# ubiquity6/MVSNet

Hardware: AMD Instinct MI355X
Metric: depth maps/sec (N=5, D=192, 160x128) (higher is better)
Workload: dtype f32; 1 GPU; M: features->depth, N=5 views, D=192 planes, 160x128 feature maps, C=32, 3D-CNN regulariser (RegNetUS0), network_mode=normal; one reference view per step per GPU, sharded by reference view; conv_impl=auto, streams_per_gpu=1

## Files before the change

include/mvsnet_hip.h:

```cpp
#ifndef MVSNET_HIP_H_
#define MVSNET_HIP_H_

#include <stddef.h>
#include <stdint.h>

#ifdef __cplusplus
extern "C" {
#endif

#define MVS_ABI_VERSION 1

#define MVS_E_BADARG   (-1)
#define MVS_E_SHAPE    (-2)
#define MVS_E_WORKSPACE (-3)
#define MVS_E_NOT_PREPARED (-4)
#define MVS_E_NO_SLOT  (-5)

#define MVS_CONV_IMPL_AUTO   0
#define MVS_CONV_IMPL_SCALAR 1
#define MVS_CONV_IMPL_MFMA   2
#define MVS_CONV_IMPL_BF16X3 3

int mvs_abi_version(void);
const char* mvs_error_string(int code);
int mvs_set_conv_impl(int impl);
int mvs_get_conv_impl(void);

#define MVS_HOOK_CV_TILE_ROWS_LOG2    0
#define MVS_HOOK_CONV_NO_SPAN         1
#define MVS_HOOK_CONV_NO_FUSE2        2
#define MVS_HOOK_S2_PLANES            3
#define MVS_HOOK_GRU_ONE_STREAM       4
#define MVS_HOOK_GRU_PRODUCER_THREADS 5
#define MVS_HOOK_UNET_PERSISTENT       6
#define MVS_HOOK_UNET_GRID            7
#define MVS_HOOK_FUSE2_PLANES          8
#define MVS_HOOK_REGNET_SIDE_BRANCH    9
#define MVS_HOOK_OUT_PLANES           10
#define MVS_HOOK_BN_SLOTS             11
#define MVS_HOOK_PAIR_SLOTS           12
#define MVS_HOOK_CONV_FULL_SWEEPS     13
#define MVS_HOOK_PAIR_PLANES          14
#define MVS_HOOK_S1_PLANES            15
#define MVS_HOOK_SPAN_FORCE           16
#define MVS_HOOK_PAIR_DIRECT          17
#define MVS_HOOK_PAIR_WAVES4          18
#define MVS_HOOK_COUNT                19
int mvs_set_test_hook(int id, int value);
int mvs_get_test_hook(int id);

int mvs_homography_transforms_f32(const float* cams, int view_num, int depth_num,
                                  float depth_start, float depth_interval, float depth_end,
                                  int inverse_depth, float* homographies, float* transforms,
                                  void* stream);

int mvs_cost_volume_f32(const float* ref, const float* src, const float* transforms,
                        int view_num, int depth_total, int d_begin, int d_count,
                        int H, int W, int C, int variant, int negate, int border,
                        float* cost, void* stream);

int mvs_warp_f32(const float* image, const float* transform8, int H, int W, int C, int border,
                 float* out, void* stream);

int mvs_conv3d_f32(const float* x, const float* x_scale, const float* x_shift,
                   const float* x2, const float* x2_scale, const float* x2_shift,
                   const float* w, int D, int H, int W, int Cin, int Cout, int stride,
                   float* y, double* stats, void* stream);
int mvs_deconv3d_f32(const float* x, const float* x_scale, const float* x_shift,
                     const float* x2, const float* x2_scale, const float* x2_shift,
                     const float* w, int D, int H, int W, int Cin, int Cout,
                     float* y, double* stats, void* stream);

int mvs_conv3d_pair_f32(const float* x, const float* w1, const float* w2, int D, int H, int W,
                        int Cin, int Cout1, int Cout2, float* y1, double* stats1,
                        float* y2, double* stats2, void* stream);

int mvs_bn_finalize_f32(const double* stats, int C, double count, const float* gamma,
                        const float* beta, float eps, float* scale, float* shift, void* stream);
int mvs_zero_f64(double* p, size_t n, void* stream);

size_t mvs_regnet_workspace_bytes(int D, int H, int W, int cin, int base);
size_t mvs_regnet_prepared_floats(int cin, int base);
int mvs_regnet_prepare_f32(const float* const* weights, int cin, int base, float* prepared,
                           void* stream);
int mvs_regnet_us0_prepared_f32(const float* cost, int D, int H, int W, int cin, int base,
                                const float* const* weights, const float* prepared,
                                const float* const* gammas, const float* const* betas, float eps,
                                void* workspace, size_t workspace_bytes, float* reg, void* stream);

int mvs_gn_stat_slots(void);
size_t mvs_conv2d_prepared_floats(int ks, int cin1, int cin2, int cout);
int mvs_conv2d_prepare_f32(const float* w, int ks, int cin1, int cin2, int cout, float* prepared, void* stream);
int mvs_conv2d_prepare_dgrad_f32(const float* w, int ks, int cin_fwd, int cout_fwd, float* prepared, void* stream);
int mvs_conv2d_gn_f32(const float* x1, const double* stats1, const float* gamma1, const float* beta1, int c1, int relu1,
                      const float* x2, const double* stats2, const float* gamma2, const float* beta2, int c2, int relu2,
                      const float* prepared, int V, int H, int W, int cout, int ks, int stride,
                      float* y, double* stats_out, void* stream);
int mvs_unet_prepare_many_f32(int n, const int* kind, const float* const* w, const int* ks, const int* c1, const int* c2,
                              const int* cin_src, const int* cout, float* const* prepared, void* stream);
size_t mvs_deconv2d_prepared_floats(int cin, int cout);
int mvs_deconv2d_prepare_f32(const float* w, int cin, int cout, float* prepared, void* stream);
int mvs_deconv2d_gn_f32(const float* x, const double* stats, const float* gamma, const float* beta, int cin, int relu,
                        const float* w, const float* prepared, int V, int H, int W, int cout, float* y,
                        double* stats_out, void* stream);

size_t mvs_center_images_workspace_bytes(int V);
int mvs_center_images_u8_f32(const uint8_t* images, int V, int H, int W, float* out4, void* workspace, void* stream);

int mvs_profile_dominant(int enable);
int mvs_profile_dominant_ms(double* avg_ms, int* count);
int mvs_profile_stages(int enable);
int mvs_profile_stages_ms(double* avg_ms3, int* count);
int mvs_profile_layers(int enable);
int mvs_profile_layers_ms(double* avg_ms11, int* count);
int mvs_regnet_filler_shares(int* permille3);
int mvs_depth_from_features_f32(const float* features, const float* cams, int view_num, int depth_num,
                                int H, int W, int C, int base, float depth_start, float depth_interval,
                                float depth_end, int inverse_depth, int variant,
                                const float* const* weights, const float* prepared,
                                const float* const* gammas, const float* const* betas, float eps,
                                float* transforms, float* cost, void* workspace, size_t workspace_bytes,
                                float* reg, float* depth, float* prob, void* stream);
int mvs_regnet_us0_batch_f32(const float* cost, int batch, int D, int H, int W, int cin, int base,
                             const float* const* weights, const float* prepared,
                             const float* const* gammas, const float* const* betas, float eps,
                             void* workspace, size_t workspace_bytes, float* reg, void* stream);
int mvs_regnet_us0_f32(const float* cost, int D, int H, int W, int cin, int base,
                       const float* const* weights, const float* const* gammas,
                       const float* const* betas, float eps, void* workspace,
                       size_t workspace_bytes, float* reg, void* stream);

int mvs_softargmin_prob_f32(const float* reg, int D, int H, int W, float depth_start,
                            float depth_interval, int inverse_depth, float* depth, float* prob,
                            void* stream);

int mvs_conv2d_cat_f32(const float* xa, int Ca, const float* xb, int Cb, const float* w,
                       const float* bias, int H, int W, int Cout, float* y, double* stats,
                       int groups, void* stream);

int mvs_gru_gates_f32(const float* g, const double* stats, const float* reset_gamma,
                      const float* reset_beta, const float* update_gamma, const float* update_beta,
                      const float* h, int H, int W, int F, float* rh, float* u, void* stream);
int mvs_gru_blend_f32(const float* c, const double* stats, const float* out_gamma,
                      const float* out_beta, const float* u, int H, int W, int F, float* h,
                      void* stream);

int mvs_wta_update_f32(const float* reg, float depth_value, int H, int W, float* max_prob,
                       float* depth_image, float* exp_sum, void* stream);
int mvs_wta_finish_f32(const float* max_prob, const float* exp_sum, int H, int W, float* prob_out,
                       void* stream);

size_t mvs_gru_workspace_bytes(int H, int W, int C, int f1, int f2, int f3);
int mvs_gru_wta_f32(const float* ref, const float* src, const float* transforms, int view_num,
                    int depth_num, int H, int W, int C, int f1, int f2, int f3,
                    const float* const* params, const float* depth_values, void* workspace,
                    size_t workspace_bytes, float* depth_out, float* prob_out, void* stream);

int mvs_gru_fused_route(int C, int f1, int f2, int f3, size_t view_block_bytes);
int mvs_gru_wta_batch_f32(const float* const* ref, const float* const* src, const float* const* transforms,
                          int views, int view_num, int depth_num, int H, int W, int C, int f1, int f2,
                          int f3, const float* const* params, const float* depth_values, void* workspace,
                          size_t workspace_bytes, float* depth_out, float* prob_out, void* stream);

int mvs_gru_prepare(void* stream);
int mvs_gru_release(void* stream);

int mvs_gru_set_formulation(int form);

int mvs_gru_fused_trace(void* buffer, int capacity);

int mvs_gru_stream_layout(void* stream, int* pipe_of_caller, float* probe_us);

int mvs_softargmin_bwd_f32(const float* reg, const float* g_depth, const float* g_prob, int D, int H, int W,
                           float depth_start, float depth_interval, int inverse_depth,
                           float* g_reg, void* stream);
int mvs_bn_relu_f32(const float* y, const float* scale, const float* shift, const float* y2,
                    const float* scale2, const float* shift2, size_t voxels, int C, float* out,
                    void* stream);
int mvs_bn_bwd_sum_slots(void);
int mvs_bn_bwd_reduce_f32(const float* y, const double* stats, double count, float eps,
                          const float* scale, const float* shift, const float* g1,
                          const float* g2, size_t voxels, int C, double* sums, void* stream);
int mvs_bn_bwd_apply_f32(const float* y, const double* stats, double count, float eps,
                         const float* scale, const float* shift, const float* gamma,
                         const float* g1, const float* g2, const double* sums, size_t voxels,
                         int C, float* g_y, float* g_gamma, float* g_beta, void* stream);
size_t mvs_conv3d_wgrad_workspace_bytes(int D, int H, int W, int Cbig, int Csmall, int stride);
int mvs_conv3d_wgrad_f32(const float* big, const float* small, int D, int H, int W, int Cbig,
                         int Csmall, int stride, void* workspace, size_t workspace_bytes,
                         float* dw, void* stream);
int mvs_cost_volume_bwd_f32(const float* ref, const float* src, const float* transforms,
                            int view_num, int depth_num, int H, int W, int C, const float* g1,
                            const float* g2, float* g_ref, float* g_src, void* stream);
size_t mvs_cost_volume_bwd_workspace_bytes(int view_num, int depth_num, int H, int W, int C);
int mvs_cost_volume_bwd_gather_f32(const float* ref, const float* src, const float* transforms,
                                   int view_num, int depth_num, int H, int W, int C, const float* g1,
                                   const float* g2, void* workspace, size_t workspace_bytes,
                                   float* g_ref, float* g_src, void* stream);
int mvs_rmsprop_step_f32(float* w, const float* g, float* ms, float* mom, size_t n, float lr,
                         float decay, float momentum, float eps, float grad_scale, void* stream);
int mvs_gn_stats_f32(const float* x, int V, size_t hw, int C, double* stats, void* stream);
int mvs_gn_slots_to_channel_sums_f64(const double* slots, int V, int C, int nslot, double* stats, void* stream);
int mvs_gn_slots_to_channel_sums_many_f64(int n, const double* slots, const long long* slot_off, const int* C, int V, int nslot,
                                          double* stats, const long long* stat_off, void* stream);
int mvs_gn_apply_f32(const float* x, const double* stats, const float* gamma, const float* beta, float eps,
                     int relu, int V, size_t hw, int C, float* y, void* stream);
int mvs_gn_bwd_sum_slots(void);
size_t mvs_gn_bwd_sums_doubles(int V, int C);
int mvs_gn_bwd_reduce_f32(const float* x, const double* stats, const float* gamma, const float* beta, float eps,
                          int relu, const float* g, int V, size_t hw, int C, double* sums, void* stream);
int mvs_gn_bwd_apply_f32(const float* x, const double* stats, const float* gamma, const float* beta, float eps,
                         int relu, const float* g, const double* sums, int V, size_t hw, int C, float* dx,
                         void* stream);
int mvs_gn_bwd_apply_tot_f32(const float* x, const double* stats, const float* gamma, const float* beta, float eps,
                             int relu, const float* g, const double* sums, double* totals, int V, size_t hw, int C, float* dx,
                             void* stream);
int mvs_momentum_step_f32(float* w, const float* g, float* accum, size_t n, float lr, float momentum,
                          float grad_scale, void* stream);
int mvs_adam_step_f32(float* w, const float* g, float* m, float* v, size_t n, float lr_t, float beta1,
                      float beta2, float eps, float grad_scale, void* stream);

int mvs_transpose_add_many_f32(int n, const float* const* src, float* const* dst, const int* dims, void* stream);
int mvs_add_f64_many_f32(int n, const double* const* src, float* const* dst, const int* counts, void* stream);
int mvs_add_many_f32(int n, const float* const* src, float* const* dst, const long long* counts, void* stream);

int mvs_gru_train_slots(int* forward_slots, int* backward_slots);
int mvs_gru_train_cell_fwd_f32(const float* px, const float* wgh, const float* woh, const float* ln, int D, int H,
                               int W, int F, float* g, float* c, float* rh, float* h, double* stats, void* stream);
int mvs_gru_train_cell_bwd_f32(const float* gh, const float* g, const float* c, const float* h, const double* stats,
                               const float* wgh_t, const float* woh_t, const float* ln, int D, int H, int W, int F,
                               float* gpx, double* part, float* scratch, const float* dh_in, float* dh_out,
                               void* stream);

size_t mvs_conv2d_wgrad_workspace_bytes(int N, int H, int W, int Cin, int Cout);
int mvs_conv2d_wgrad_f32(const float* x, const float* g, int g_stride, int g_off, int N, int H, int W, int Cin,
                         int Cout, void* workspace, size_t workspace_bytes, float* dw, void* stream);

size_t mvs_fusion_workspace_bytes(int V, int H, int W, int max_sources, int dedupe);
int mvs_fusion_f32(const float* depth, const float* prob, int V, int H, int W, const float* tables, const int* src_offsets,
                   const int* src_index, int max_sources, float prob_threshold, float reproj_threshold,
                   float depth_rel_threshold, float num_consistent, int dedupe, const uint8_t* images, int img_h, int img_w,
                   float* xyz, uint8_t* rgb, int* view_index, int* pixel_index, int* count, void* workspace,
                   size_t workspace_bytes, void* stream);

int mvs_depth_normals_f32(const float* depth, const float* prob, int V, int H, int W, const float* tables, float prob_threshold,
                          float jump_threshold, float* normals, void* stream);
size_t mvs_fusion_normals_workspace_bytes(int V, int H, int W, int max_sources, int dedupe);
int mvs_fusion_normals_f32(const float* depth, const float* prob, int V, int H, int W, const float* tables,
                           const int* src_offsets, const int* src_index, int max_sources, float prob_threshold,
                           float reproj_threshold, float depth_rel_threshold, float num_consistent, int dedupe,
                           float jump_threshold, float normal_cos_threshold, const uint8_t* images, int img_h, int img_w,
                           float* xyz, uint8_t* rgb, float* normals, int* view_index, int* pixel_index, int* count,
                           void* workspace, size_t workspace_bytes, void* stream);

size_t mvs_nn_workspace_bytes(int n_query, int n_target, int gx, int gy, int gz);
int mvs_nn_f32(const float* query, int n_query, const float* target, int n_target, float ox, float oy, float oz, float cell,
               int gx, int gy, int gz, float max_dist, float* dist, int* index, void* workspace, size_t workspace_bytes,
               void* stream);
int mvs_nn_query_f32(int n_query, int n_target, float ox, float oy, float oz, float cell, int gx, int gy, int gz,
                     float max_dist, float* dist, int* index, int* visited, const void* workspace, size_t workspace_bytes,
                     void* stream);
size_t mvs_nn_target_workspace_bytes(int n_target, int gx, int gy, int gz);
int mvs_nn_target_build_f32(const float* target, int n_target, float ox, float oy, float oz, float cell, int gx, int gy, int gz,
                            void* workspace, size_t workspace_bytes, void* stream);
size_t mvs_icp_step_workspace_bytes(int n_source);
int mvs_icp_step_f32(const float* source, int n_source, const int* order, const double* T, const double* cp, const double* cq,
                     float ox, float oy, float oz, float cell, int gx, int gy, int gz, int n_target,
                     const void* target_workspace, size_t target_workspace_bytes, float max_corr_dist, double* moments,
                     float* dist, int* index, void* workspace, size_t workspace_bytes, void* stream);
size_t mvs_dist_stats_workspace_bytes(int n, int n_thresholds);
int mvs_dist_stats_f32(const float* dist, int n, float max_dist, const float* thresholds, int n_thresholds, double* out,
                       void* workspace, size_t workspace_bytes, void* stream);
int mvs_voxel_keys_f32(const float* xyz, int n, double min_x, double min_y, double min_z, double cell, long long* keys,
                       void* stream);
size_t mvs_voxel_select_workspace_bytes(int n);
int mvs_voxel_select_f32(const float* xyz, int n, const long long* sorted_keys, const long long* order, float* out, int* count,
                         void* workspace, size_t workspace_bytes, void* stream);

size_t mvs_render_workspace_bytes(int V, int H, int W, int occlusion);
int mvs_render_points_f32(const float* xyz, int n, const int* order, const float* proj, int V, int H, int W, int splat,
                          float min_depth, int occl_radius, float occl_ratio, int occl_count, float* depth, int* index,
                          void* workspace, size_t workspace_bytes, void* stream);

int mvs_view_visibility_f32(const float* xyz, int n, const float* proj, const int* view_bits, int V, int H, int W,
                            float min_depth, const float* zbuf, float z_tol, unsigned long long* mask, int mask_words,
                            void* stream);
size_t mvs_view_scores_workspace_bytes(int n, int V);
int mvs_view_scores_f32(const float* xyz, int n, const int* order, const unsigned long long* mask, int mask_words,
                        const float* centres, int V, const unsigned short* table, long long* score_sum, long long* shared,
                        void* workspace, size_t workspace_bytes, void* stream);
int mvs_view_depth_hist_f32(const float* xyz, int n, const float* proj, int V, const unsigned long long* mask, int mask_words,
                            int pass, const int* prefixes, unsigned int* hist, void* stream);

size_t mvs_tsdf_integrate_workspace_bytes(int V, int H, int W);
int mvs_tsdf_integrate_f32(const float* depth, const float* prob, int V, int H, int W, const float* proj,
                           const unsigned char* images, int img_h, int img_w, const float* origin, float voxel, int nx, int ny,
                           int nz, float trunc, float prob_threshold, int flags, float* sum, int* count, unsigned int* rgb_sum,
                           int* rgb_count, void* workspace, size_t workspace_bytes, void* stream);
size_t mvs_surface_nets_workspace_bytes(int nx, int ny, int nz);
int mvs_surface_nets_count_f32(const float* sum, const int* count, int nx, int ny, int nz, int min_count, int* totals,
                               void* workspace, size_t workspace_bytes, void* stream);
int mvs_surface_nets_write_f32(const float* sum, const int* count, const unsigned int* rgb_sum, const int* rgb_count,
                               const float* origin, float voxel, int nx, int ny, int nz, int min_count, const int* cell_rank,
                               const int* face_end, int M, int F, float* vertices, unsigned char* colours, int* faces,
                               void* workspace, size_t workspace_bytes, void* stream);

size_t mvs_raster_workspace_bytes(int V, int H, int W, int queue_capacity);
int mvs_raster_mesh_f32(const float* vertices, int M, const int* faces, int F, const int* order, const float* proj, int V,
                        int H, int W, float min_depth, int cull, int large_pixels, int queue_capacity, float* depth,
                        int* index, void* workspace, size_t workspace_bytes, void* stream);
int mvs_raster_interpolate_f32(const float* vertices, int M, const int* faces, int F, const float* proj, int V, int H, int W,
                               float min_depth, const int* index, const float* attr, int C, float* out, void* stream);

size_t mvs_mesh_components_workspace_bytes(long long M, long long F);
int mvs_mesh_components_label_i32(const float* vertices, long long M, const int* faces, long long F, int* vertex_labels,
                                  int* face_labels, void* workspace, size_t workspace_bytes, void* stream);
int mvs_mesh_components_measure_f32(const float* vertices, long long M, long long F, const int* vertex_labels,
                                    const int* face_labels, int* counts, unsigned int* boxes, void* workspace,
                                    size_t workspace_bytes, void* stream);
int mvs_mesh_compact_mark_i32(const int* faces, long long M, long long F, const int* face_labels, const int* keep_label,
                              int* face_keep, int* vertex_keep, void* stream);
int mvs_mesh_compact_write_f32(const float* vertices, const unsigned char* colours, long long M, const int* faces, long long F,
                               const int* face_keep, const int* face_rank, const int* vertex_keep, const int* vertex_rank,
                               long long M_out, long long F_out, float* out_vertices, unsigned char* out_colours, int* out_faces,
                               void* stream);

size_t mvs_mesh_cluster_workspace_bytes(long long M, long long F);
int mvs_mesh_cluster_keys_f32(const float* vertices, long long M, const int* faces, long long F, float origin_x, float origin_y,
                              float origin_z, float cell, long long* keys, int* offsets, void* workspace, size_t workspace_bytes,
                              void* stream);
int mvs_mesh_cluster_heads_i64(const long long* sorted_keys, long long M, int* head, void* stream);
int mvs_mesh_cluster_sums_f32(const long long* sorted_keys, const long long* order, const int* head_rank, const int* offsets,
                              const unsigned char* colours, long long M, float origin_x, float origin_y, float origin_z,
                              float cell, int* vertex_cluster, float* cluster_vertices, unsigned char* cluster_colours,
                              void* workspace, size_t workspace_bytes, void* stream);
int mvs_mesh_cluster_faces_i32(const int* faces, long long M, long long F, const int* vertex_cluster, int* cluster_faces,
                               long long* key_lo, long long* key_hi, void* workspace, size_t workspace_bytes, void* stream);
int mvs_mesh_cluster_mark_i32(const int* cluster_faces, long long M, long long F, const long long* sorted_lo,
                              const long long* sorted_hi, const long long* order, int* face_keep, int* vertex_keep,
                              void* workspace, size_t workspace_bytes, void* stream);

size_t mvs_mesh_sample_workspace_bytes(long long M, long long F);
int mvs_mesh_sample_quota_f32(const float* vertices, long long M, const int* faces, long long F, double density, long long* quota,
                              void* workspace, size_t workspace_bytes, void* stream);
int mvs_mesh_sample_write_f32(const float* vertices, const unsigned char* colours, long long M, const int* faces, long long F,
                              const long long* sums, long long N, unsigned long long seed, float* out_xyz, int* out_face,
                              unsigned char* out_colours, float* out_normals, void* stream);

#ifdef __cplusplus
}
#endif
#endif
```

mvsnet_amd/_lib.py:

```python
from __future__ import annotations

import ctypes as C
import os

import torch

_HERE = os.path.dirname(os.path.abspath(__file__))
LIB_PATH = os.environ.get("MVS_LIB_PATH") or os.path.join(_HERE, "libmvsnet_hip.so")

_f = C.c_float
_i = C.c_int
_p = C.c_void_p
_sz = C.c_size_t
_pp = C.POINTER(C.c_void_p)
_ll = C.c_longlong

SIGNATURES = {
    "mvs_abi_version": (_i, []),
    "mvs_error_string": (C.c_char_p, [_i]),
    "mvs_set_conv_impl": (_i, [_i]),
    "mvs_get_conv_impl": (_i, []),
    "mvs_homography_transforms_f32": (_i, [_p, _i, _i, _f, _f, _f, _i, _p, _p, _p]),
    "mvs_cost_volume_f32": (_i, [_p, _p, _p, _i, _i, _i, _i, _i, _i, _i, _i, _i, _i, _p, _p]),
    "mvs_warp_f32": (_i, [_p, _p, _i, _i, _i, _i, _p, _p]),
    "mvs_conv3d_f32": (_i, [_p] * 7 + [_i] * 6 + [_p, _p, _p]),
    "mvs_deconv3d_f32": (_i, [_p] * 7 + [_i] * 5 + [_p, _p, _p]),
    "mvs_conv3d_pair_f32": (_i, [_p] * 3 + [_i] * 6 + [_p] * 5),
    "mvs_gn_stat_slots": (_i, []),
    "mvs_conv2d_prepared_floats": (_sz, [_i, _i, _i, _i]),
    "mvs_conv2d_prepare_f32": (_i, [_p, _i, _i, _i, _i, _p, _p]),
    "mvs_conv2d_prepare_dgrad_f32": (_i, [_p, _i, _i, _i, _p, _p]),
    "mvs_conv2d_gn_f32": (_i, [_p, _p, _p, _p, _i, _i, _p, _p, _p, _p, _i, _i, _p, _i, _i, _i, _i, _i, _i, _p, _p, _p]),
    "mvs_deconv2d_prepared_floats": (_sz, [_i, _i]),
    "mvs_deconv2d_prepare_f32": (_i, [_p, _i, _i, _p, _p]),
    "mvs_deconv2d_gn_f32": (_i, [_p, _p, _p, _p, _i, _i, _p, _p, _i, _i, _i, _i, _p, _p, _p]),
    "mvs_profile_dominant": (_i, [_i]),
    "mvs_profile_dominant_ms": (_i, [_p, _p]),
    "mvs_profile_stages": (_i, [_i]),
    "mvs_profile_stages_ms": (_i, [_p, _p]),
    "mvs_profile_layers": (_i, [_i]),
    "mvs_profile_layers_ms": (_i, [_p, _p]),
    "mvs_bn_finalize_f32": (_i, [_p, _i, C.c_double, _p, _p, _f, _p, _p, _p]),
    "mvs_zero_f64": (_i, [_p, _sz, _p]),
    "mvs_regnet_workspace_bytes": (_sz, [_i, _i, _i, _i, _i]),
    "mvs_regnet_us0_f32": (_i, [_p, _i, _i, _i, _i, _i, _pp, _pp, _pp, _f, _p, _sz, _p, _p]),
    "mvs_regnet_prepared_floats": (_sz, [_i, _i]),
    "mvs_regnet_prepare_f32": (_i, [_pp, _i, _i, _p, _p]),
    "mvs_depth_from_features_f32": (_i, [_p, _p, _i, _i, _i, _i, _i, _i, _f, _f, _f, _i, _i, _pp, _p, _pp, _pp, _f,
                                         _p, _p, _p, _sz, _p, _p, _p, _p]),
    "mvs_regnet_us0_batch_f32": (_i, [_p, _i, _i, _i, _i, _i, _i, _pp, _p, _pp, _pp, _f, _p, _sz, _p, _p]),
    "mvs_regnet_us0_prepared_f32": (_i, [_p, _i, _i, _i, _i, _i, _pp, _p, _pp, _pp, _f, _p, _sz, _p, _p]),
    "mvs_softargmin_prob_f32": (_i, [_p, _i, _i, _i, _f, _f, _i, _p, _p, _p]),
    "mvs_conv2d_cat_f32": (_i, [_p, _i, _p, _i, _p, _p, _i, _i, _i, _p, _p, _i, _p]),
    "mvs_gru_gates_f32": (_i, [_p] * 7 + [_i, _i, _i, _p, _p, _p]),
    "mvs_gru_blend_f32": (_i, [_p] * 5 + [_i, _i, _i, _p, _p]),
    "mvs_wta_update_f32": (_i, [_p, _f, _i, _i, _p, _p, _p, _p]),
    "mvs_wta_finish_f32": (_i, [_p, _p, _i, _i, _p, _p]),
    "mvs_gru_workspace_bytes": (_sz, [_i] * 6),
    "mvs_softargmin_bwd_f32": (_i, [_p, _p, _p, _i, _i, _i, _f, _f, _i, _p, _p]),
    "mvs_bn_relu_f32": (_i, [_p] * 6 + [_sz, _i, _p, _p]),
    "mvs_bn_bwd_sum_slots": (_i, []),
    "mvs_bn_bwd_reduce_f32": (_i, [_p, _p, C.c_double, _f, _p, _p, _p, _p, _sz, _i, _p, _p]),
    "mvs_bn_bwd_apply_f32": (_i, [_p, _p, C.c_double, _f, _p, _p, _p, _p, _p, _p, _sz, _i, _p, _p, _p, _p]),
    "mvs_conv3d_wgrad_workspace_bytes": (_sz, [_i] * 6),
    "mvs_conv3d_wgrad_f32": (_i, [_p, _p] + [_i] * 6 + [_p, _sz, _p, _p]),
    "mvs_cost_volume_bwd_f32": (_i, [_p, _p, _p] + [_i] * 5 + [_p, _p, _p, _p, _p]),
    "mvs_cost_volume_bwd_workspace_bytes": (_sz, [_i] * 5),
    "mvs_cost_volume_bwd_gather_f32": (_i, [_p, _p, _p] + [_i] * 5 + [_p, _p, _p, _sz, _p, _p, _p]),
    "mvs_rmsprop_step_f32": (_i, [_p, _p, _p, _p, _sz, _f, _f, _f, _f, _f, _p]),
    "mvs_gn_stats_f32": (_i, [_p, _i, _sz, _i, _p, _p]),
    "mvs_unet_prepare_many_f32": (_i, [_i, _p, _p, _p, _p, _p, _p, _p, _p, _p]),
    "mvs_transpose_add_many_f32": (_i, [_i, _p, _p, _p, _p]),
    "mvs_add_f64_many_f32": (_i, [_i, _p, _p, _p, _p]),
    "mvs_add_many_f32": (_i, [_i, _p, _p, _p, _p]),
    "mvs_center_images_workspace_bytes": (_sz, [_i]),
    "mvs_center_images_u8_f32": (_i, [_p, _i, _i, _i, _p, _p, _p]),
    "mvs_gn_slots_to_channel_sums_many_f64": (_i, [_i, _p, _p, _p, _i, _i, _p, _p, _p]),
    "mvs_gn_bwd_sums_doubles": (_sz, [_i, _i]),
    "mvs_gn_slots_to_channel_sums_f64": (_i, [_p, _i, _i, _i, _p, _p]),
    "mvs_gn_apply_f32": (_i, [_p, _p, _p, _p, _f, _i, _i, _sz, _i, _p, _p]),
    "mvs_gn_bwd_reduce_f32": (_i, [_p, _p, _p, _p, _f, _i, _p, _i, _sz, _i, _p, _p]),
    "mvs_gn_bwd_apply_f32": (_i, [_p, _p, _p, _p, _f, _i, _p, _p, _i, _sz, _i, _p, _p]),
    "mvs_gn_bwd_apply_tot_f32": (_i, [_p, _p, _p, _p, _f, _i, _p, _p, _p, _i, _sz, _i, _p, _p]),
    "mvs_gn_bwd_sum_slots": (_i, []),
    "mvs_momentum_step_f32": (_i, [_p, _p, _p, _sz, _f, _f, _f, _p]),
    "mvs_adam_step_f32": (_i, [_p, _p, _p, _p, _sz, _f, _f, _f, _f, _f, _p]),
    "mvs_gru_train_slots": (_i, [C.POINTER(C.c_int), C.POINTER(C.c_int)]),
    "mvs_gru_train_cell_fwd_f32": (_i, [_p, _p, _p, _p, _i, _i, _i, _i, _p, _p, _p, _p, _p, _p]),
    "mvs_gru_train_cell_bwd_f32": (_i, [_p, _p, _p, _p, _p, _p, _p, _p, _i, _i, _i, _i, _p, _p, _p, _p, _p, _p]),
    "mvs_conv2d_wgrad_workspace_bytes": (_sz, [_i] * 5),
    "mvs_conv2d_wgrad_f32": (_i, [_p, _p, _i, _i, _i, _i, _i, _i, _i, _p, _sz, _p, _p]),
    "mvs_gru_wta_f32": (_i, [_p, _p, _p] + [_i] * 8 + [_pp, C.POINTER(C.c_float), _p, _sz, _p, _p, _p]),
    "mvs_gru_wta_batch_f32": (_i, [_pp, _pp, _pp] + [_i] * 9 + [_pp, C.POINTER(C.c_float), _p, _sz, _p, _p, _p]),
    "mvs_gru_set_formulation": (_i, [_i]),
    "mvs_gru_fused_route": (_i, [_i, _i, _i, _i, _sz]),
    "mvs_set_test_hook": (_i, [_i, _i]),
    "mvs_get_test_hook": (_i, [_i]),
    "mvs_gru_fused_trace": (_i, [_p, _i]),
    "mvs_gru_prepare": (_i, [_p]),
    "mvs_gru_release": (_i, [_p]),
    "mvs_gru_stream_layout": (_i, [_p, C.POINTER(C.c_int), C.POINTER(C.c_float)]),
    "mvs_regnet_filler_shares": (_i, [C.POINTER(C.c_int)]),
    "mvs_mesh_cluster_workspace_bytes": (_sz, [_ll, _ll]),
    "mvs_mesh_cluster_keys_f32": (_i, [_p, _ll, _p, _ll, _f, _f, _f, _f, _p, _p, _p, _sz, _p]),
    "mvs_mesh_cluster_heads_i64": (_i, [_p, _ll, _p, _p]),
    "mvs_mesh_cluster_sums_f32": (_i, [_p, _p, _p, _p, _p, _ll, _f, _f, _f, _f, _p, _p, _p, _p, _sz, _p]),
    "mvs_mesh_cluster_faces_i32": (_i, [_p, _ll, _ll, _p, _p, _p, _p, _p, _sz, _p]),
    "mvs_mesh_cluster_mark_i32": (_i, [_p, _ll, _ll, _p, _p, _p, _p, _p, _p, _sz, _p]),
    "mvs_mesh_sample_workspace_bytes": (_sz, [_ll, _ll]),
    "mvs_mesh_sample_quota_f32": (_i, [_p, _ll, _p, _ll, C.c_double, _p, _p, _sz, _p]),
    "mvs_mesh_sample_write_f32": (_i, [_p, _p, _ll, _p, _ll, _p, _ll, C.c_ulonglong, _p, _p, _p, _p, _p]),
    "mvs_fusion_workspace_bytes": (_sz, [_i] * 5),
    "mvs_fusion_f32": (_i, [_p, _p, _i, _i, _i, _p, _p, _p, _i, _f, _f, _f, _f, _i, _p, _i, _i, _p, _p, _p, _p, _p, _p, _sz, _p]),
    "mvs_depth_normals_f32": (_i, [_p, _p, _i, _i, _i, _p, _f, _f, _p, _p]),
    "mvs_fusion_normals_workspace_bytes": (_sz, [_i] * 5),
    "mvs_fusion_normals_f32": (_i, [_p, _p, _i, _i, _i, _p, _p, _p, _i, _f, _f, _f, _f, _i, _f, _f, _p, _i, _i, _p, _p, _p, _p, _p,
                                    _p, _p, _sz, _p]),
    "mvs_nn_workspace_bytes": (_sz, [_i] * 5),
    "mvs_nn_f32": (_i, [_p, _i, _p, _i, _f, _f, _f, _f, _i, _i, _i, _f, _p, _p, _p, _sz, _p]),
    "mvs_nn_query_f32": (_i, [_i, _i, _f, _f, _f, _f, _i, _i, _i, _f, _p, _p, _p, _p, _sz, _p]),
    "mvs_nn_target_workspace_bytes": (_sz, [_i] * 4),
    "mvs_nn_target_build_f32": (_i, [_p, _i, _f, _f, _f, _f, _i, _i, _i, _p, _sz, _p]),
    "mvs_icp_step_workspace_bytes": (_sz, [_i]),
    "mvs_icp_step_f32": (_i, [_p, _i, _p, C.POINTER(C.c_double), C.POINTER(C.c_double), C.POINTER(C.c_double), _f, _f, _f, _f,
                              _i, _i, _i, _i, _p, _sz, _f, _p, _p, _p, _p, _sz, _p]),
    "mvs_dist_stats_workspace_bytes": (_sz, [_i, _i]),
    "mvs_dist_stats_f32": (_i, [_p, _i, _f, C.POINTER(C.c_float), _i, _p, _p, _sz, _p]),
    "mvs_voxel_keys_f32": (_i, [_p, _i, C.c_double, C.c_double, C.c_double, C.c_double, _p, _p]),
    "mvs_voxel_select_workspace_bytes": (_sz, [_i]),
    "mvs_voxel_select_f32": (_i, [_p, _i, _p, _p, _p, _p, _p, _sz, _p]),
    "mvs_render_workspace_bytes": (_sz, [_i] * 4),
    "mvs_render_points_f32": (_i, [_p, _i, _p, _p, _i, _i, _i, _i, _f, _i, _f, _i, _p, _p, _p, _sz, _p]),
    "mvs_view_visibility_f32": (_i, [_p, _i, _p, _p, _i, _i, _i, _f, _p, _f, _p, _i, _p]),
    "mvs_view_scores_workspace_bytes": (_sz, [_i, _i]),
    "mvs_view_scores_f32": (_i, [_p, _i, _p, _p, _i, _p, _i, _p, _p, _p, _p, _sz, _p]),
    "mvs_view_depth_hist_f32": (_i, [_p, _i, _p, _i, _p, _i, _i, _p, _p, _p]),
    "mvs_tsdf_integrate_workspace_bytes": (_sz, [_i] * 3),
    "mvs_tsdf_integrate_f32": (_i, [_p, _p, _i, _i, _i, _p, _p, _i, _i, C.POINTER(C.c_float), _f, _i, _i, _i, _f, _f, _i, _p, _p, _p,
                                    _p, _p, _sz, _p]),
    "mvs_surface_nets_workspace_bytes": (_sz, [_i] * 3),
    "mvs_surface_nets_count_f32": (_i, [_p, _p, _i, _i, _i, _i, _p, _p, _sz, _p]),
    "mvs_surface_nets_write_f32": (_i, [_p, _p, _p, _p, C.POINTER(C.c_float), _f, _i, _i, _i, _i, _p, _p, _i, _i, _p, _p, _p, _p, _sz,
                                        _p]),
    "mvs_raster_workspace_bytes": (_sz, [_i] * 4),
    "mvs_raster_mesh_f32": (_i, [_p, _i, _p, _i, _p, _p, _i, _i, _i, _f, _i, _i, _i, _p, _p, _p, _sz, _p]),
    "mvs_raster_interpolate_f32": (_i, [_p, _i, _p, _i, _p, _i, _i, _i, _f, _p, _p, _i, _p, _p]),
    "mvs_mesh_components_workspace_bytes": (_sz, [_ll, _ll]),
    "mvs_mesh_components_label_i32": (_i, [_p, _ll, _p, _ll, _p, _p, _p, _sz, _p]),
    "mvs_mesh_components_measure_f32": (_i, [_p, _ll, _ll, _p, _p, _p, _p, _p, _sz, _p]),
    "mvs_mesh_compact_mark_i32": (_i, [_p, _ll, _ll, _p, _p, _p, _p, _p]),
    "mvs_mesh_compact_write_f32": (_i, [_p, _p, _ll, _p, _ll, _p, _p, _p, _p, _ll, _ll, _p, _p, _p, _p]),
}

CONV_IMPL = {"auto": 0, "scalar": 1, "mfma": 2, "bf16x3": 3}
HOOKS = {"cv_tile_rows_log2": 0, "conv_no_span": 1, "conv_no_fuse2": 2, "s2_planes": 3, "gru_one_stream": 4,
         "gru_producer_threads": 5, "unet_persistent": 6, "unet_grid": 7, "fuse2_planes": 8, "regnet_side_branch": 9,
         "out_planes": 10, "bn_slots": 11, "pair_slots": 12, "conv_full_sweeps": 13, "pair_planes": 14, "s1_planes": 15,
         "span_force": 16, "pair_direct": 17, "pair_waves4": 18}
HOOK_DEFAULTS = {"cv_tile_rows_log2": -1, "conv_no_span": 0, "conv_no_fuse2": 0, "s2_planes": 0, "gru_one_stream": 0,
                 "gru_producer_threads": 128, "unet_persistent": 1, "unet_grid": 0, "fuse2_planes": 0, "regnet_side_branch": 0,
                 "out_planes": 0, "bn_slots": 0, "pair_slots": 0, "conv_full_sweeps": 0, "pair_planes": 0, "s1_planes": 0,
                 "span_force": 0, "pair_direct": 0, "pair_waves4": 0}

_lib = None


class MvsnetHipError(RuntimeError):
    pass


def load():
    global _lib
    if _lib is None:
        if not os.path.exists(LIB_PATH):
            raise MvsnetHipError(
                "libmvsnet_hip.so not found at %s -- build it with `python -m mvsnet_amd.build` "
                "(there is no CPU fallback)" % LIB_PATH)
        lib = C.CDLL(LIB_PATH)
        for name, (res, args) in SIGNATURES.items():
            fn = getattr(lib, name)
            fn.restype = res
            fn.argtypes = args
        if lib.mvs_abi_version() != 1:
            raise MvsnetHipError("libmvsnet_hip.so ABI version mismatch")
        _lib = lib
    return _lib


def check(rc: int, what: str = ""):
    if rc != 0:
        msg = load().mvs_error_string(rc).decode()
        raise MvsnetHipError("%s failed: %s (code %d)" % (what or "mvsnet_hip call", msg, rc))


def ptr(t):
    if t is None:
        return None
    if not t.is_cuda:
        raise MvsnetHipError("expected a device tensor (no CPU path exists)")
    if not t.is_contiguous():
        raise MvsnetHipError("expected a contiguous tensor")
    cur = torch.cuda.current_device()
    if t.device.index != cur:
        raise MvsnetHipError("tensor is on cuda:%s but the current device is cuda:%d -- call "
                             "torch.cuda.set_device (mvsnet_amd.shard.bind_device) before any library call"
                             % (t.device.index, cur))
    return C.c_void_p(t.data_ptr())


def f32(t, name="tensor"):
    if t.dtype != torch.float32:
        raise MvsnetHipError("%s must be float32, got %s" % (name, t.dtype))
    return t


def stream_ptr():
    return C.c_void_p(torch.cuda.current_stream().cuda_stream)


def gpu_ready():
    try:
        load()
    except Exception as e:
        return str(e)
    if not torch.cuda.is_available():
        return "no GPU is visible to this process"
    return None


def device(device, what):
    dev = torch.device(device) if device is not None else torch.device("cuda")
    if dev.type != "cuda":
        raise ValueError("%s runs on a GPU device, got %s" % (what, dev))
    if not torch.cuda.is_available():
        raise MvsnetHipError("%s runs on the GPU (HIP); no GPU is visible to this process" % what)
    return dev if dev.index is not None else torch.device("cuda", torch.cuda.current_device())


import threading

_GRU_LOCK = threading.Lock()
_GRU_PREPARED = {}
_GRU_NO_SLOT = set()
_GRU_GENERATION = [0]
MVS_E_NO_SLOT = -5


def gru_prepare():
    key = (torch.cuda.current_device(), int(torch.cuda.current_stream().cuda_stream))
    if torch.cuda.is_current_stream_capturing():
        return None
    with _GRU_LOCK:
        if key in _GRU_NO_SLOT:
            return None
        if key not in _GRU_PREPARED:
            rc = load().mvs_gru_prepare(stream_ptr())
            if rc == MVS_E_NO_SLOT:
                _GRU_NO_SLOT.add(key)
                import warnings
                warnings.warn("mvsnet_amd: all 16 stream sets of mvs_gru_prepare are in use; the recurrent sweep of this stream runs on the "
                              "stream alone (drop DepthPlan objects of streams you no longer use, or call _lib.gru_release())", RuntimeWarning)
                return None
            check(rc, "mvs_gru_prepare")
            _GRU_GENERATION[0] += 1
            _GRU_PREPARED[key] = [_GRU_GENERATION[0], 0]
        _GRU_PREPARED[key][1] += 1
        return key + (_GRU_PREPARED[key][0],)


def gru_unref(token):
    if token is None:
        return
    key, gen = token[:2], token[2]
    with _GRU_LOCK:
        ent = _GRU_PREPARED.get(key)
        if ent is None or ent[0] != gen:
            return
        ent[1] -= 1
        if ent[1] > 0:
            return
        del _GRU_PREPARED[key]
        _GRU_NO_SLOT.clear()
        try:
            with torch.cuda.device(key[0]):
                load().mvs_gru_release(C.c_void_p(key[1]))
        except Exception:
            pass


def gru_release():
    key = (torch.cuda.current_device(), int(torch.cuda.current_stream().cuda_stream))
    with _GRU_LOCK:
        if key in _GRU_PREPARED:
            del _GRU_PREPARED[key]
            _GRU_NO_SLOT.clear()
            check(load().mvs_gru_release(stream_ptr()), "mvs_gru_release")


def ptr_array(tensors):
    arr = (C.c_void_p * len(tensors))()
    for k, t in enumerate(tensors):
        arr[k] = ptr(t).value if t is not None else None
    return arr


def set_conv_impl(name: str):
    check(load().mvs_set_conv_impl(CONV_IMPL[name]), "mvs_set_conv_impl")


def set_test_hook(name: str, value: int):
    check(load().mvs_set_test_hook(HOOKS[name], int(value)), "mvs_set_test_hook(%s, %d)" % (name, value))


class test_hooks:

    def __init__(self, **kw):
        self.kw = kw

    def __enter__(self):
        for k, v in self.kw.items():
            set_test_hook(k, v)
        return self

    def __exit__(self, *exc):
        for k in self.kw:
            set_test_hook(k, HOOK_DEFAULTS[k])
        return False
```

mvsnet_amd/build.py:

```python
from __future__ import annotations

import os
import subprocess
import sys
from concurrent.futures import ThreadPoolExecutor

HERE = os.path.dirname(os.path.abspath(__file__))
CSRC = os.path.join(HERE, "csrc")
LIB_PATH = os.path.join(HERE, "libmvsnet_hip.so")
SOURCES = ["homography.hip", "cost_volume.hip", "conv3d_scalar.hip", "conv3d_mfma.hip", "conv3d_s2_mfma.hip",
           "deconv3d_mfma.hip", "deconv3d_c8.hip", "conv3d_os.hip", "conv3d_out.hip", "conv3d_bf16x3.hip", "conv3d_c8.hip", "conv3d_c8_wino.hip",
           "regnet.hip", "library.hip", "softargmin.hip", "gru.hip", "gru_mfma.hip", "gru_fused.hip", "gru_streams.hip", "gru_sweep.hip", "unet2d.hip", "unet2d_p.hip", "center_images.hip", "multi_tensor.hip",
           "backward.hip", "groupnorm.hip", "optimizer.hip", "conv3d_wgrad.hip", "conv3d_c1.hip", "conv3d_k8.hip", "gru_train.hip", "conv2d_wgrad.hip",
           "fusion.hip", "pointcloud.hip", "render.hip", "view_selection.hip", "tsdf.hip", "raster.hip", "mesh_components.hip", "mesh_simplify.hip", "mesh_sample.hip"]
HIPCC = os.environ.get("HIPCC", "/opt/rocm/bin/hipcc")
FLAGS = ["--offload-arch=gfx950", "-O3", "-std=c++17", "-fPIC", "-Wall", "-Wno-unused-function"]
FLAGS += os.environ.get("MVS_EXTRA_HIPCC_FLAGS", "").split()


def _stale(out, deps):
    if not os.path.exists(out):
        return True
    t = os.path.getmtime(out)
    return any(os.path.getmtime(d) > t for d in deps)


def build_library(force=False, verbose=True):
    headers = [os.path.join(CSRC, "common.h"),
               os.path.join(HERE, "..", "include", "mvsnet_hip.h")]
    headers += [os.path.join(CSRC, f) for f in os.listdir(CSRC) if f.endswith(".h")]
    objs, jobs = [], []
    for s in SOURCES:
        src = os.path.join(CSRC, s)
        obj = os.path.join(CSRC, s.replace(".hip", ".o"))
        objs.append(obj)
        if force or _stale(obj, [src] + headers):
            jobs.append([HIPCC] + FLAGS + ["-c", src, "-o", obj])

    def run(cmd):
        if verbose:
            print(" ".join(cmd), flush=True)
        r = subprocess.run(cmd, capture_output=True, text=True)
        if r.returncode != 0:
            raise RuntimeError("hipcc failed:\n%s\n%s" % (r.stdout, r.stderr))
        if verbose and r.stderr.strip():
            print(r.stderr, file=sys.stderr)

    if jobs:
        with ThreadPoolExecutor(max_workers=min(4, len(jobs))) as ex:
            list(ex.map(run, jobs))
    if jobs or force or _stale(LIB_PATH, objs):
        run([HIPCC, "--offload-arch=gfx950", "-shared", "-fPIC", "-o", LIB_PATH] + objs)
    return LIB_PATH


LAB_LIB_PATH = os.path.join(HERE, "variants", "libmvsnet_lab.so")
LAB_SOURCES = ["cost_volume_lds.hip", "cost_volume_mfma.hip"]


def build_lab(verbose=True):
    os.makedirs(os.path.dirname(LAB_LIB_PATH), exist_ok=True)
    lab = os.path.join(CSRC, "lab")
    deps = [os.path.join(CSRC, f) for f in os.listdir(CSRC) if f.endswith(".h")]
    objs = []
    for s_ in LAB_SOURCES:
        src, obj = os.path.join(lab, s_), os.path.join(lab, s_.replace(".hip", ".o"))
        objs.append(obj)
        if _stale(obj, [src] + deps):
            cmd = [HIPCC] + FLAGS + ["-c", src, "-o", obj]
            if verbose:
                print(" ".join(cmd), flush=True)
            r = subprocess.run(cmd, capture_output=True, text=True)
            if r.returncode != 0:
                raise RuntimeError("hipcc failed:\n%s\n%s" % (r.stdout, r.stderr))
    if _stale(LAB_LIB_PATH, objs):
        r = subprocess.run([HIPCC, "--offload-arch=gfx950", "-shared", "-fPIC", "-o", LAB_LIB_PATH] + objs, capture_output=True, text=True)
        if r.returncode != 0:
            raise RuntimeError("link failed:\n%s\n%s" % (r.stdout, r.stderr))
    return LAB_LIB_PATH


if __name__ == "__main__":
    if "--lab" in sys.argv:
        print(build_lab())
    else:
        print(build_library(force="--force" in sys.argv))
```

mvsnet_amd/csrc/conv3d_c8_wino.hip:

```cpp
#include "conv_common.h"
#include <cstdlib>
#include <cstdio>

namespace {

constexpr int TW = 32;
constexpr int TH = 8;
constexpr int PW = TW + 2;
constexpr int HP = PW / 2;
constexpr int CIN = 32, COUT = 8, CQ = CIN / 4;
constexpr int COUT2 = 16;
constexpr int NPOS = (TH + 2) * PW;
constexpr int NF4 = NPOS * CQ;
constexpr int NROWS = 3 * COUT;
constexpr int WROW = NROWS * 4;
constexpr int NPT = 4;
constexpr int W_FLOATS = 3 * NPT * CQ * WROW;
constexpr int SP = CIN;
constexpr int ROWP = PW * SP;
constexpr int SLAB_FLOATS = NPOS * SP;
constexpr int KH_FLOATS = NPT * CQ * WROW;
constexpr int NCT = 4;
constexpr int RED_FLOATS = 3 * NCT * 64 * 4;
constexpr int LDS_FLOATS = 2 * SLAB_FLOATS + W_FLOATS + 4 + RED_FLOATS;
constexpr int SLOTS = 256;

typedef float f32x2 __attribute__((ext_vector_type(2)));
typedef unsigned int u32x4_t __attribute__((ext_vector_type(4)));
constexpr int OOB = (int)0x80000000u;

__device__ __forceinline__ int slab_off(int row, int col, int slot) {
    const int pc = (col & 1) * HP + (col >> 1);
    return (row * PW + pc) * SP + (((slot + 2 * (pc >> 1)) & 7) << 2);
}

__device__ __forceinline__ float wino_u(float g0, float g1, float g2, int pt) {
    if (pt == 0) return g0;
    if (pt == 3) return g2;
    const double s = (double)g0 + (double)g2;
    return (float)(0.5 * (pt == 1 ? s + (double)g1 : s - (double)g1));
}
__device__ __forceinline__ float wino_weight(const float* __restrict__ w, int i) {
    const int j = i & 3;
    const int r = (i >> 2) % NROWS;
    const int g = (i >> 2) / NROWS;
    const int ciq = g % CQ, tap = g / CQ;
    const int kh = tap >> 2, pt = tap & 3;
    const int kd = r / COUT, co = r - kd * COUT;
    const float* p = w + ((size_t)((kd * 3 + kh) * 3) * CIN + ciq * 4 + j) * COUT + co;
    return wino_u(p[0], p[CIN * COUT], p[2 * CIN * COUT], pt);
}

__global__ void wino_weight_layout_kernel(const float* __restrict__ w, float* __restrict__ out) {
    const int i = blockIdx.x * blockDim.x + threadIdx.x;
    if (i < W_FLOATS) out[i] = wino_weight(w, i);
}

struct WinoArgs {
    const float* wprep;
    const float* w2;
    float* y2;
    double* stats2;
    int slots1, slots2;
    int span_g, span_m;
    int span_b[17];
    int full_sweeps;
};

template <bool SPAN, bool W8>
__global__ void __launch_bounds__(W8 ? 512 : 256, 1)
conv3d_c8_wino_kernel(ConvArgs a, WinoArgs fa) {
    extern __shared__ __attribute__((aligned(16))) float smem[];
    float* slab = smem;
    float* wl = smem + 2 * SLAB_FLOATS;
    float* red = wl + W_FLOATS + 4;
    constexpr int ZOFF = W_FLOATS;

    const int tid = threadIdx.x;
    const int lane = tid & 63, wave = __builtin_amdgcn_readfirstlane(tid >> 6);
    const int rw = W8 ? wave & 3 : wave;
    const int n = lane & 15, kq = lane >> 4;

    const int tiles_w = (a.W + TW - 1) / TW;
    int seg_tile[2], seg_d0[2], seg_d1[2], nseg = 1;
    if (SPAN) {
        const int per_xcd = gridDim.x >> 3, j = blockIdx.x >> 3, x = blockIdx.x & 7;
        const int lin = (gridDim.x & 7) ? (int)blockIdx.x : x * per_xcd + j;
        const int grp = lin / fa.span_m, k = lin - grp * fa.span_m;
        const int lo = fa.span_b[k], hi_ = fa.span_b[k + 1];
        const int t0 = lo / a.D, t1 = (hi_ - 1) / a.D;
        seg_tile[0] = grp * fa.span_g + t0; seg_d0[0] = lo - t0 * a.D; seg_d1[0] = min(hi_, (t0 + 1) * a.D) - t0 * a.D;
        seg_tile[1] = grp * fa.span_g + t1; seg_d0[1] = 0; seg_d1[1] = hi_ - t1 * a.D;
        nseg = t1 != t0 ? 2 : 1;
    } else {
        seg_tile[0] = xcd_swizzle(blockIdx.x, gridDim.x);
        seg_d0[0] = blockIdx.z * a.planes_per_wg;
        seg_d1[0] = min(seg_d0[0] + a.planes_per_wg, a.D);
        seg_tile[1] = 0; seg_d0[1] = 0; seg_d1[1] = 0;
    }
    int h0 = (seg_tile[0] / tiles_w) * TH, w0 = (seg_tile[0] % tiles_w) * TW;
    int d0 = seg_d0[0], d1 = seg_d1[0];
    int T = d1 - d0 + 2;

    auto init_weights = [&]() __attribute__((always_inline)) {
        if (fa.wprep) copy_weights_to_lds(wl, fa.wprep, W_FLOATS);
        else for (int i = tid; i < W_FLOATS; i += 256) wl[i] = wino_weight(a.w, i);
        if (tid < 4) wl[ZOFF + tid] = 0.f;
    };

    constexpr int NTH = W8 ? 512 : 256, NITW = (NF4 + NTH - 1) / NTH;
    const int c4 = tid % CQ;
    float4 pre[NITW];
    int goff[NITW], loff[NITW];
    auto set_goff = [&]() __attribute__((always_inline)) {
#pragma unroll
        for (int i = 0; i < NITW; ++i) {
            int f = tid + NTH * i;
            if (f >= NF4) f -= NTH;
            int pos = f / CQ;
            int r = pos / PW, c = pos - r * PW;
            int gh = h0 - 1 + r, gw = w0 - 1 + c;
            bool inb = gh >= 0 && gh < a.H && gw >= 0 && gw < a.W;
            goff[i] = inb ? ((gh * a.W + gw) * CIN + 4 * c4) * 4 : OOB;
            loff[i] = slab_off(r, c, c4);
        }
    };
    const int plane_bytes = a.H * a.W * CIN * 4;
    const auto xrsrc = __builtin_amdgcn_make_buffer_rsrc((void*)a.x, 0, a.D * plane_bytes, 0x00020000);
    const auto yrsrc = __builtin_amdgcn_make_buffer_rsrc((void*)a.y, 0, a.D * a.H * a.W * COUT * 4, 0x00020000);

    auto load_piece = [&](int i, int q) __attribute__((always_inline)) {
        const bool plane_ok = (q >= 0) && (q < a.D);
        u32x4_t v = __builtin_amdgcn_raw_buffer_load_b128(xrsrc, goff[i] | (plane_ok ? 0 : OOB),
                                                           plane_ok ? q * plane_bytes : 0, 0);
        pre[i] = make_float4(__uint_as_float(v[0]), __uint_as_float(v[1]), __uint_as_float(v[2]), __uint_as_float(v[3]));
    };
    auto stage_piece = [&](int i, float* buf) __attribute__((always_inline)) {
        *(float4*)(buf + loff[i]) = pre[i];
    };

    f32x4 acc[NPT][3];
#pragma unroll
    for (int p = 0; p < NPT; ++p)
#pragma unroll
        for (int i = 0; i < 3; ++i) acc[p][i] = (f32x4){0.f, 0.f, 0.f, 0.f};
    float st_s[4] = {0.f, 0.f, 0.f, 0.f}, st_q[4] = {0.f, 0.f, 0.f, 0.f};

    int bcol[4];
#pragma unroll
    for (int c = 0; c < 4; ++c) bcol[c] = slab_off(2 * rw, 2 * n + c, kq);
    const int hi = n >> 3;
    const int a_lane = (kq * NROWS + (n & 7)) * 4;

    auto sweep = [&](auto Pc, auto Mc, const float* buf, auto&& extra) __attribute__((always_inline)) {
        constexpr int P = decltype(Pc)::value, TM = decltype(Mc)::value;
        constexpr int KD_B0 = P % 3, KD_B1 = (P + 2) % 3, KD_B2 = (P + 1) % 3;
        const int a0 = a_lane + (hi ? KD_B1 : KD_B0) * COUT * 4;
        const int ap = a_lane + KD_B2 * COUT * 4 - hi * KH_FLOATS;
        f32x4 da[2], db[2], pv[2], av[3];
        auto load_grp = [&](int G, int r) __attribute__((always_inline)) {
            const int i = G & 3, pt = G >> 3, s = (G >> 2) & 1;
            const int wconst = (pt * CQ + 4 * s) * WROW;
            if (r == 0) {
                const int ca = pt == 0 ? 0 : pt == 2 ? 2 : 1, cb = pt == 0 ? 2 : pt == 1 ? 2 : pt == 2 ? 1 : 3;
                da[G & 1] = *(const f32x4*)(buf + (bcol[ca] ^ (16 * s)) + i * ROWP);
                db[G & 1] = *(const f32x4*)(buf + (bcol[cb] ^ (16 * s)) + i * ROWP);
            } else if (r == 1) {
                int off = ap + i * KH_FLOATS + wconst;
                if (i == 0) off = hi ? ZOFF : off;
                if (i == 3) off = hi ? off : ZOFF;
                pv[G & 1] = *(const f32x4*)(wl + off);
            } else if (i < 3) av[i] = *(const f32x4*)(wl + a0 + i * KH_FLOATS + wconst);
        };
        constexpr int NG = 8 * NPT;
        f32x4 bt[2];
        auto form = [&](int G) __attribute__((always_inline)) {
            bt[G & 1] = (G >> 3) == 1 ? da[G & 1] + db[G & 1] : da[G & 1] - db[G & 1];
        };
#pragma unroll
        for (int r = 0; r < 3; ++r) load_grp(0, r);
        form(0);
#pragma unroll
        for (int G = 0; G < NG; ++G) {
            const int i = G & 3, pt = G >> 3;
            const int NC = (i == 0 || i == 3) ? 2 : 3;
#pragma unroll
            for (int j = 0; j < 4; ++j) {
#pragma unroll
                for (int c = 0; c < NC; ++c) {
                    int t; float aval;
                    if (c == NC - 1) { t = 2; aval = pv[G & 1][j]; }
                    else if (i == 0) { t = 0; aval = av[0][j]; }
                    else if (c == 0) { t = 1; aval = av[i - 1][j]; }
                    else { t = 0; aval = av[i][j]; }
                    if ((TM >> t) & 1) acc[pt][t] = __builtin_amdgcn_mfma_f32_16x16x4f32(aval, bt[G & 1][j], acc[pt][t], 0, 0, 0);
                }
                if (G + 1 < NG) {
                    if (j == 0) load_grp(G + 1, 0);
                    if (j == 1) { load_grp(G + 1, 1); load_grp(G + 1, 2); }
                    if (j == 2) form(G + 1);
                }
                if (j == 3) extra(G);
                __builtin_amdgcn_sched_barrier(0);
            }
        }
    };

    int yoff[3];
    auto set_yoff = [&]() __attribute__((always_inline)) {
        const int w = w0 + 2 * n, co = 4 * (kq & 1);
        const int hs[3] = {h0 + 2 * rw, h0 + 2 * rw + 1, h0 + 2 * rw + (kq >> 1)};
#pragma unroll
        for (int i = 0; i < 3; ++i)
            yoff[i] = (hs[i] < a.H && w < a.W) ? ((hs[i] * a.W + w) * COUT + co) * 4 : OOB;
    };
    const int yplane_bytes = a.H * a.W * COUT * 4;
    auto retire = [&](auto Pc, int o) __attribute__((always_inline)) {
        constexpr int P = decltype(Pc)::value;
        constexpr int B = (P + 1) % 3;
        const bool plane_ok = (o >= d0) && (o < d1);
        auto emit = [&](int t, int yo) __attribute__((always_inline)) {
            if (plane_ok) {
                const f32x4 m0 = acc[0][t], m1 = acc[1][t], m2 = acc[2][t], m3 = acc[3][t];
                f32x4 y[2];
                y[0] = (m0 + m1) + m2;
                y[1] = (m1 - m2) - m3;
#pragma unroll
                for (int e = 0; e < 2; ++e) {
                    u32x4_t v = {__float_as_uint(y[e][0]), __float_as_uint(y[e][1]), __float_as_uint(y[e][2]), __float_as_uint(y[e][3])};
                    __builtin_amdgcn_raw_buffer_store_b128(v, yrsrc, yo + e * COUT * 4 + o * yplane_bytes, 0, 0);
                    if (yo >= 0) {
#pragma unroll
                        for (int k = 0; k < 4; ++k) { st_s[k] += y[e][k]; st_q[k] = __builtin_fmaf(y[e][k], y[e][k], st_q[k]); }
                    }
                }
            }
#pragma unroll
            for (int p = 0; p < NPT; ++p) acc[p][t] = (f32x4){0.f, 0.f, 0.f, 0.f};
        };
        if (B < 2) {
            if ((kq >> 1) == B) { emit(0, yoff[0]); emit(1, yoff[1]); }
        } else {
            emit(2, yoff[2]);
        }
    };

    float wS[3][9][2];
    f32x4 cur[NCT], prv[NCT];
    int s2b[3][2];
    float st2_s[4] = {0.f, 0.f, 0.f, 0.f}, st2_q[4] = {0.f, 0.f, 0.f, 0.f};
    int fin_od = -1;
    const int Ho = a.H / 2, Wo = a.W / 2;
    auto init_s2 = [&]() __attribute__((always_inline)) {
#pragma unroll
        for (int kd = 0; kd < 3; ++kd)
#pragma unroll
            for (int tap = 0; tap < 9; ++tap)
#pragma unroll
                for (int j = 0; j < 2; ++j)
                    wS[kd][tap][j] = fa.w2[((size_t)(kd * 9 + tap) * CIN + 8 * rw + 2 * kq + j) * COUT2 + n];
#pragma unroll
        for (int kw = 0; kw < 3; ++kw)
#pragma unroll
            for (int wt = 0; wt < 2; ++wt)
                s2b[kw][wt] = slab_off(2 * (n >> 3), 16 * wt + 2 * (n & 7) + kw + 1, 2 * rw + (kq >> 1)) + 2 * (kq & 1);
#pragma unroll
        for (int ct = 0; ct < NCT; ++ct) { cur[ct] = (f32x4){0.f, 0.f, 0.f, 0.f}; prv[ct] = cur[ct]; }
    };

    auto s2_sweep = [&](auto Ec, const float* buf, auto&& extra2) __attribute__((always_inline)) {
        constexpr int MODE = decltype(Ec)::value;
        f32x2 b2[2][NCT];
        auto ld = [&](int tap, f32x2 (&b)[NCT]) __attribute__((always_inline)) {
            const int kh = tap / 3, kw = tap % 3;
#pragma unroll
            for (int ct = 0; ct < NCT; ++ct) b[ct] = *(const f32x2*)(buf + s2b[kw][ct & 1] + (4 * (ct >> 1) + kh + 1) * ROWP);
        };
        ld(0, b2[0]);
#pragma unroll
        for (int tap = 0; tap < 9; ++tap) {
            if (tap + 1 < 9) ld(tap + 1, b2[(tap + 1) & 1]);
#pragma unroll
            for (int j = 0; j < 2; ++j)
#pragma unroll
                for (int ct = 0; ct < NCT; ++ct) {
                    const float bval = b2[tap & 1][ct][j];
                    if (MODE) {
                        if (MODE == 1) cur[ct] = __builtin_amdgcn_mfma_f32_16x16x4f32(wS[0][tap][j], bval, cur[ct], 0, 0, 0);
                        prv[ct] = __builtin_amdgcn_mfma_f32_16x16x4f32(wS[2][tap][j], bval, prv[ct], 0, 0, 0);
                    } else {
                        cur[ct] = __builtin_amdgcn_mfma_f32_16x16x4f32(wS[1][tap][j], bval, cur[ct], 0, 0, 0);
                    }
                }
            extra2(tap);
            __builtin_amdgcn_sched_barrier(0);
        }
    };
    auto s2_park = [&](int od) __attribute__((always_inline)) {
        if (rw > 0) {
#pragma unroll
            for (int ct = 0; ct < NCT; ++ct)
                *(f32x4*)(red + (((rw - 1) * NCT + ct) * 64 + lane) * 4) = prv[ct];
        }
        fin_od = od;
    };
    auto s2_finish = [&]() __attribute__((always_inline)) {
        if (fin_od >= 0 && rw == 0) {
#pragma unroll
            for (int ct = 0; ct < NCT; ++ct) {
                f32x4 r = prv[ct];
#pragma unroll
                for (int w = 0; w < 3; ++w) {
                    f32x4 p = *(const f32x4*)(red + ((w * NCT + ct) * 64 + lane) * 4);
                    r[0] += p[0]; r[1] += p[1]; r[2] += p[2]; r[3] += p[3];
                }
                const int oh = h0 / 2 + 2 * (ct >> 1) + (n >> 3), ow = w0 / 2 + 8 * (ct & 1) + (n & 7);
                if (oh < Ho && ow < Wo) {
                    float* dst = fa.y2 + ((((size_t)fin_od * Ho + oh) * Wo) + ow) * COUT2 + 4 * kq;
                    *(float4*)dst = make_float4(r[0], r[1], r[2], r[3]);
#pragma unroll
                    for (int k = 0; k < 4; ++k) { st2_s[k] += r[k]; st2_q[k] = __builtin_fmaf(r[k], r[k], st2_q[k]); }
                }
            }
        }
        fin_od = -1;
    };

    auto march = [&](auto Rc) __attribute__((always_inline)) {
        constexpr int ROLE = decltype(Rc)::value;
        constexpr bool S1 = ROLE != 2, S2 = ROLE != 1;
        if (S1) {
            init_weights();
            set_yoff();
        }
        set_goff();
        if (S2) init_s2();

        auto prologue = [&](int t0) __attribute__((always_inline)) {
            float* buf = slab + (t0 & 1) * SLAB_FLOATS;
#pragma unroll
            for (int i = 0; i < NITW; ++i) load_piece(i, d0 - 1 + t0);
#pragma unroll
            for (int i = 0; i < NITW; ++i) stage_piece(i, buf);
#pragma unroll
            for (int i = 0; i < NITW; ++i) load_piece(i, d0 + t0);
            __syncthreads();
        };
        auto stage_item = [&](int k, float* nxt, int q) __attribute__((always_inline)) {
            if (k < NITW) stage_piece(k, nxt); else load_piece(k - NITW, q + 2);
        };
        auto stage_all = [&](float* nxt, int q) __attribute__((always_inline)) {
#pragma unroll
            for (int k = 0; k < 2 * NITW; ++k) stage_item(k, nxt, q);
        };

        auto plane = [&](auto Pc, int t) __attribute__((always_inline)) {
            const int q = d0 - 1 + t;
            float* cur_buf = slab + (t & 1) * SLAB_FLOATS;
            float* nxt = slab + ((t + 1) & 1) * SLAB_FLOATS;
            const bool in_vol = (q >= 0) && (q < a.D);
            auto extra = [&](int G) __attribute__((always_inline)) {
                if (S1) {
                    if (G >= 4 && G < 4 + NITW) stage_piece(G - 4, nxt);
                    if (G >= 16 && G < 16 + NITW) load_piece(G - 16, q + 2);
                }
            };
            auto extra2 = [&](int tap) __attribute__((always_inline)) {
                if (ROLE == 2) {
#pragma unroll
                    for (int k = 0; k < 2 * NITW; ++k)
                        if (k >= tap * 2 * NITW / 9 && k < (tap + 1) * 2 * NITW / 9) stage_item(k, nxt, q);
                }
            };
            if (S2) s2_finish();
            if (S1) sweep(Pc, std::integral_constant<int, 7>{}, cur_buf, extra);
            if (S2) {
                const bool even = q >= d0 && !(q & 1);
                const bool swept = q >= d0 && in_vol;
                if (even) {
#pragma unroll
                    for (int ct = 0; ct < NCT; ++ct) { prv[ct] = cur[ct]; cur[ct] = (f32x4){0.f, 0.f, 0.f, 0.f}; }
                }
                if (swept) {
                    if (q & 1) s2_sweep(std::false_type{}, cur_buf, extra2);
                    else s2_sweep(std::true_type{}, cur_buf, extra2);
                } else if (ROLE == 2) {
                    stage_all(nxt, q);
                }
                if (even) {
                    const int od_prev = q / 2 - 1;
                    if (2 * od_prev >= d0) s2_park(od_prev);
                }
            }
            if (S1) retire(Pc, q - 1);
            __syncthreads();
        };
        auto first_plane = [&]() __attribute__((always_inline)) {
            const int q = d0 - 1;
            float* nxt = slab + SLAB_FLOATS;
            auto extra = [&](int G) __attribute__((always_inline)) {
                if (S1) {
                    if (G >= 4 && G < 4 + NITW) stage_piece(G - 4, nxt);
                    if (G >= 16 && G < 16 + NITW) load_piece(G - 16, q + 2);
                }
            };
            if (S1) {
                sweep(std::integral_constant<int, 0>{}, std::integral_constant<int, 3>{}, slab, extra);
                retire(std::integral_constant<int, 0>{}, q - 1);
            }
            if (ROLE == 2) stage_all(nxt, q);
            __syncthreads();
        };
        auto last_plane = [&](auto Pc) __attribute__((always_inline)) {
            constexpr int P = decltype(Pc)::value;
            const int q = d1;
            const float* cur_buf = slab + ((T - 1) & 1) * SLAB_FLOATS;
            const bool in_vol = q < a.D;
            if (S2) s2_finish();
            if (S1 && in_vol) sweep(Pc, std::integral_constant<int, (P + 1) % 3 == 2 ? 4 : 3>{}, cur_buf, [](int) {});
            if (S2) {
#pragma unroll
                for (int ct = 0; ct < NCT; ++ct) { prv[ct] = cur[ct]; cur[ct] = (f32x4){0.f, 0.f, 0.f, 0.f}; }
                if (in_vol) s2_sweep(std::integral_constant<int, 2>{}, cur_buf, [](int) {});
                const int od_prev = q / 2 - 1;
                if (2 * od_prev >= d0) s2_park(od_prev);
            }
            if (S1) retire(Pc, q - 1);
            __syncthreads();
        };
        for (int sg = 0; sg < (SPAN ? nseg : 1); ++sg) {
            if (SPAN && sg > 0) {
                if (S2) s2_finish();
                h0 = (seg_tile[1] / tiles_w) * TH; w0 = (seg_tile[1] % tiles_w) * TW;
                d0 = seg_d0[1]; d1 = seg_d1[1]; T = d1 - d0 + 2;
                set_goff();
                if (S1) {
                    set_yoff();
#pragma unroll
                    for (int p = 0; p < NPT; ++p)
#pragma unroll
                        for (int i = 0; i < 3; ++i) acc[p][i] = (f32x4){0.f, 0.f, 0.f, 0.f};
                }
                if (S2) {
#pragma unroll
                    for (int ct = 0; ct < NCT; ++ct) { cur[ct] = (f32x4){0.f, 0.f, 0.f, 0.f}; prv[ct] = cur[ct]; }
                }
            }
            const bool trim_first = fa.full_sweeps == 0 || (fa.full_sweeps == 2 && d0 == 0);
            const bool trim_last = fa.full_sweeps == 0 || (fa.full_sweeps == 2 && d1 == a.D);
            const int t_lo = trim_first ? 1 : 0, t_hi = trim_last ? T - 1 : T;
            prologue(trim_first && d0 == 0 ? 1 : 0);
            if (trim_first && d0 > 0) first_plane();
            for (int t = 0; t < t_hi; t += 3) {
                if (t >= t_lo) plane(std::integral_constant<int, 0>{}, t);
                if (t + 1 < t_hi) plane(std::integral_constant<int, 1>{}, t + 1);
                if (t + 2 < t_hi) plane(std::integral_constant<int, 2>{}, t + 2);
            }
            if (trim_last) {
                const int pl = (T - 1) % 3;
                if (pl == 0) last_plane(std::integral_constant<int, 0>{});
                else if (pl == 1) last_plane(std::integral_constant<int, 1>{});
                else last_plane(std::integral_constant<int, 2>{});
            }
        }
        if (S2) {
            s2_finish();
            if (fa.stats2 && rw == 0) {
#pragma unroll
                for (int k = 0; k < 4; ++k) {
                    float sv = st2_s[k], qv = st2_q[k];
#pragma unroll
                    for (int o = 8; o > 0; o >>= 1) { sv += __shfl_xor(sv, o, 64); qv += __shfl_xor(qv, o, 64); }
                    if (n == 0) {
                        double* s2p = fa.stats2 + (size_t)((blockIdx.x + gridDim.x * blockIdx.z) % fa.slots2) * 2 * COUT2;
                        atomicAdd(&s2p[4 * kq + k], (double)sv);
                        atomicAdd(&s2p[COUT2 + 4 * kq + k], (double)qv);
                    }
                }
            }
        }
    };
    if (!W8) march(std::integral_constant<int, 0>{});
    else if (wave < 4) march(std::integral_constant<int, 1>{});
    else march(std::integral_constant<int, 2>{});

    if (a.stats) stats_commit<COUT>(st_s, st_q, true, slab,
                                    a.stats + (size_t)((blockIdx.x + gridDim.x * blockIdx.z) % fa.slots1) * 2 * COUT,
                                    a.cout_total, 0);
}

}

int mvs_conv_wino_weight_layout(const float* w, float* out, hipStream_t st) {
    wino_weight_layout_kernel<<<mvs_cdiv(W_FLOATS, 256), 256, 0, st>>>(w, out);
    return (int)hipGetLastError();
}

int mvs_conv3d_c8_wino_s2_launch(const ConvArgs& a0, const float* wprep_wino, const float* w2, float* y2, double* stats2,
                                 hipStream_t st, int slots1, int slots2) {
    ConvArgs a = a0;
    WinoArgs fa = {wprep_wino, w2, y2, stats2, slots1 > 1 ? slots1 : 1, slots2 > 1 ? slots2 : 1};
    fa.full_sweeps = mvs_hook(MVS_HOOK_CONV_FULL_SWEEPS) & 3;
    const int hk_planes = mvs_hook(MVS_HOOK_PAIR_PLANES), hk_span = mvs_hook(MVS_HOOK_SPAN_FORCE);
    if (a.x2 || a.xs || a.bn.stats || a.cout_total != COUT || (a.D & 1) || (a.H & 1) || (a.W & 1)) return MVS_E_SHAPE;
    if ((long long)a.D * a.H * a.W * CIN * 4 >= (1LL << 31)) return MVS_E_SHAPE;
    const int tiles = ((a.H + TH - 1) / TH) * ((a.W + TW - 1) / TW);
    {
        int best = 2; long long best_cost = 1LL << 60;
        for (int dr = 2; dr <= a.D; dr += 2) {
            long long wgs = (long long)tiles * ((a.D + dr - 1) / dr);
            long long cost = ((wgs + SLOTS - 1) / SLOTS) * (dr + 3);
            if (cost < best_cost) { best_cost = cost; best = dr; }
        }
        a.planes_per_wg = best;
    }
    if (hk_planes) a.planes_per_wg = hk_planes < a.D ? hk_planes : a.D;
    dim3 grid(tiles, 1, (a.D + a.planes_per_wg - 1) / a.planes_per_wg);
    const size_t smem = (size_t)LDS_FLOATS * sizeof(float);
    static bool attr_done = false;
    if (!attr_done) {
        const void* kernels[4] = {(const void*)conv3d_c8_wino_kernel<false, false>, (const void*)conv3d_c8_wino_kernel<true, false>,
                                  (const void*)conv3d_c8_wino_kernel<false, true>, (const void*)conv3d_c8_wino_kernel<true, true>};
        for (const void* k : kernels) {
            hipError_t e = hipFuncSetAttribute(k, hipFuncAttributeMaxDynamicSharedMemorySize, (int)smem);
            if (e != hipSuccess) return (int)e;
        }
        attr_done = true;
    }
    const bool w8 = !mvs_hook(MVS_HOOK_PAIR_WAVES4);
    if (!mvs_hook(MVS_HOOK_CONV_NO_SPAN) && !hk_planes) {
        const long long chunk_cost = (((long long)tiles * grid.z + SLOTS - 1) / SLOTS) * (a.planes_per_wg + 3);
        int bg = 0, bm = 0; long long bcost = chunk_cost;
        const int fg = hk_span >> 8, fm = hk_span & 255;
        for (int G = 1; G <= 8; ++G) {
            if (tiles % G || (hk_span && G != fg)) continue;
            for (int M = G; M <= 16; ++M) {
                if (hk_span && M != fm) continue;
                const int total = G * a.D;
                if (total % M || (long long)(tiles / G) * M > SLOTS) continue;
                const int L = total / M;
                if ((L & 1) || (L < 32 && !hk_span) || L > a.D) continue;
                const long long cost = L + 3 + ((a.D % L) ? 2 : 0);
                if (cost < bcost || hk_span) { bcost = cost; bg = G; bm = M; }
            }
        }
        if (bg) {
            fa.span_g = bg; fa.span_m = bm;
            for (int k = 0; k <= bm; ++k) fa.span_b[k] = k * (bg * a.D / bm);
            if (w8) conv3d_c8_wino_kernel<true, true><<<dim3((tiles / bg) * bm), 512, smem, st>>>(a, fa);
            else conv3d_c8_wino_kernel<true, false><<<dim3((tiles / bg) * bm), 256, smem, st>>>(a, fa);
            return (int)hipGetLastError();
        }
    }
    if (w8) conv3d_c8_wino_kernel<false, true><<<grid, 512, smem, st>>>(a, fa);
    else conv3d_c8_wino_kernel<false, false><<<grid, 256, smem, st>>>(a, fa);
    return (int)hipGetLastError();
}
```

mvsnet_amd/csrc/conv3d_mfma.hip:

```cpp
#include "conv_common.h"
#include <cstdlib>

namespace {

template <int CIN, int COUT, int TH, int TWG = CONV_TW> struct S1Geom {
    static constexpr bool TIGHT = (CIN == 32 && COUT == 8 && TH == 8 && TWG == CONV_TW);
    static constexpr int S = TIGHT ? CIN + 4 : SlabGeom<CIN>::S;
    static constexpr int LDS_BYTES = (9 * (CIN / 4) * 3 * COUT * 4 + 2 * (TH + 2) * (TWG + 2) * S) * 4;
    static constexpr int WGS_PER_CU = (2 * LDS_BYTES <= 160 * 1024) ? 2 : 1;
};

typedef unsigned int u32x4_t __attribute__((ext_vector_type(4)));
constexpr int OOB = (int)0x80000000u;

struct Fuse2Args {
    const float* w2;
    float* y2;
    double* stats2;
    int slots2;
    int full_sweeps;
};
constexpr int FUSE2_RED_FLOATS = 3 * 2 * 2 * 64 * 4;

template <int CIN, int COUT, int TH, bool HAS_X2, int TWG = CONV_TW, int CR = 1, bool FUSE2 = false>
__global__ void __launch_bounds__(256, (S1Geom<CIN, COUT, TH, TWG>::WGS_PER_CU))
conv3d_s1_kernel(ConvArgs a, Fuse2Args fa) {
    static_assert(!FUSE2 || (CIN == 16 && COUT == 16 && TH == 8 && TWG == CONV_TW && CR == 1 && !HAS_X2), "the fused stride-2 consumer is built for 3dconv1_1 + 3dconv2_0");
    constexpr int S = S1Geom<CIN, COUT, TH, TWG>::S;
    constexpr int PW = TWG + 2;
    constexpr int CC = 16 / CR;
    constexpr int TPR = TWG / CC;
    static_assert(TH % CR == 0 && TWG % CC == 0 && (TH * TWG) % 64 == 0, "tile must split into 4 x V column tiles");
    constexpr int NPOS = (TH + 2) * PW;
    constexpr int CQ = CIN / 4;
    constexpr int NF4 = NPOS * CQ;
    constexpr int NIT = (NF4 + 255) / 256;
    constexpr int V = TH * TWG / 64;
    constexpr int NROWS = 3 * COUT;
    constexpr int MT = (NROWS + 15) / 16;
    constexpr int WROW = NROWS * 4;
    constexpr int W_FLOATS = 9 * CQ * WROW;
    constexpr int SLAB_FLOATS = NPOS * S;
    static_assert(256 % CQ == 0, "channel quad per thread must be loop invariant");
    static_assert(NF4 >= 256, "spare threads of the last piece redo their previous one");

    extern __shared__ __attribute__((aligned(16))) float smem[];
    float* wl = smem;
    float* slab = smem + W_FLOATS;
    float* red2 = slab + 2 * SLAB_FLOATS;

    const int tid = threadIdx.x;
    const int lane = tid & 63, wave = __builtin_amdgcn_readfirstlane(tid >> 6);
    const int n = lane & 15, kq = lane >> 4;

    const int tiles_w = (a.W + TWG - 1) / TWG;
    const int bid = xcd_swizzle(blockIdx.x, gridDim.x);
    const int tile_h = bid / tiles_w, tile_w = bid - tile_h * tiles_w;
    const int h0 = tile_h * TH, w0 = tile_w * TWG;
    const int co_base = blockIdx.y * COUT;
    const int d0 = blockIdx.z * a.planes_per_wg;
    const int d1 = min(d0 + a.planes_per_wg, a.D);
    const int T = d1 - d0 + 2;
    int vrow[V], vcol[V];
#pragma unroll
    for (int v = 0; v < V; ++v) {
        const int ct = V * wave + v;
        vrow[v] = (ct / TPR) * CR + n / CC;
        vcol[v] = (ct % TPR) * CC + n % CC;
    }

    if (a.wprep) load_prepared_weights(wl, a.wprep, W_FLOATS);
    else for (int i = tid; i < W_FLOATS; i += 256) {
        int j = i & 3;
        int r = (i >> 2) % NROWS;
        int g = (i >> 2) / NROWS;
        int ciq = g % CQ, tap = g / CQ;
        int kd = r / COUT, co = r - kd * COUT;
        wl[i] = a.w[(((size_t)(kd * 9 + tap)) * CIN + ciq * 4 + j) * a.cout_total + co_base + co];
    }

    const int c4 = tid % CQ;
    float4 sc = make_float4(1.f, 1.f, 1.f, 1.f), sh = make_float4(0.f, 0.f, 0.f, 0.f);
    float4 sc2 = sc, sh2 = sh;
    const bool has_aff = a.xs != nullptr || a.bn.stats != nullptr;
    if (a.xs) { sc = *(const float4*)(a.xs + 4 * c4); sh = *(const float4*)(a.xb + 4 * c4); }
    const bool has_aff2 = HAS_X2 && (a.x2s != nullptr || a.bn2.stats != nullptr);
    if (HAS_X2 && a.x2s) { sc2 = *(const float4*)(a.x2s + 4 * c4); sh2 = *(const float4*)(a.x2b + 4 * c4); }
    __shared__ __attribute__((aligned(16))) float bn_tab[4 * CIN];
    bn_affine4_wg(a.bn, !a.xs, a.bn2, HAS_X2 && !a.x2s, bn_tab, 4 * c4, sc, sh, sc2, sh2);
    const float lo = has_aff ? 0.f : -INFINITY, lo2 = has_aff2 ? 0.f : -INFINITY;

    float4 pre[NIT];
    float4 pre2[HAS_X2 ? NIT : 1];

    int goff[NIT], loff[NIT];
#pragma unroll
    for (int i = 0; i < NIT; ++i) {
        int f = tid + 256 * i;
        if (f >= NF4) f -= 256;
        int pos = f / CQ;
        int r = pos / PW, c = pos - r * PW;
        int gh = h0 - 1 + r, gw = w0 - 1 + c;
        bool inb = gh >= 0 && gh < a.H && gw >= 0 && gw < a.W;
        goff[i] = inb ? ((gh * a.W + gw) * CIN + 4 * c4) * 4 : OOB;
        loff[i] = pos * S + 4 * c4;
    }
    const int plane_bytes = a.H * a.W * CIN * 4;
    const auto xrsrc = __builtin_amdgcn_make_buffer_rsrc((void*)a.x, 0, a.D * plane_bytes, 0x00020000);
    const auto x2rsrc = __builtin_amdgcn_make_buffer_rsrc((void*)(HAS_X2 ? a.x2 : a.x), 0, a.D * plane_bytes, 0x00020000);
    const auto yrsrc = __builtin_amdgcn_make_buffer_rsrc((void*)a.y, 0, a.D * a.H * a.W * a.cout_total * 4, 0x00020000);

    auto ld4b = [](auto rsrc, int voff, int soff) __attribute__((always_inline)) {
        u32x4_t v = __builtin_amdgcn_raw_buffer_load_b128(rsrc, voff, soff, 0);
        return make_float4(__uint_as_float(v[0]), __uint_as_float(v[1]), __uint_as_float(v[2]), __uint_as_float(v[3]));
    };
    auto load_piece = [&](int i, int q) __attribute__((always_inline)) {
        const bool plane_ok = (q >= 0) && (q < a.D);
        const int voff = goff[i] | (plane_ok ? 0 : OOB), soff = plane_ok ? q * plane_bytes : 0;
        pre[i] = ld4b(xrsrc, voff, soff);
        if (HAS_X2) pre2[i] = ld4b(x2rsrc, voff, soff);
    };
    auto stage_piece = [&](int i, int q, float* buf) __attribute__((always_inline)) {
        const bool ok = (q >= 0) && (q < a.D) && goff[i] >= 0;
        float4 v = pre[i];
        v.x = fmaxf(v.x * sc.x + sh.x, lo); v.y = fmaxf(v.y * sc.y + sh.y, lo);
        v.z = fmaxf(v.z * sc.z + sh.z, lo); v.w = fmaxf(v.w * sc.w + sh.w, lo);
        if (HAS_X2) {
            float4 u = pre2[i];
            v.x += fmaxf(u.x * sc2.x + sh2.x, lo2); v.y += fmaxf(u.y * sc2.y + sh2.y, lo2);
            v.z += fmaxf(u.z * sc2.z + sh2.z, lo2); v.w += fmaxf(u.w * sc2.w + sh2.w, lo2);
        }
        v.x = ok ? v.x : 0.f; v.y = ok ? v.y : 0.f; v.z = ok ? v.z : 0.f; v.w = ok ? v.w : 0.f;
        *(float4*)(buf + loff[i]) = v;
    };

    f32x4 acc[MT][V];
#pragma unroll
    for (int m = 0; m < MT; ++m)
#pragma unroll
        for (int v = 0; v < V; ++v) acc[m][v] = (f32x4){0.f, 0.f, 0.f, 0.f};
    float st_s[4] = {0.f, 0.f, 0.f, 0.f}, st_q[4] = {0.f, 0.f, 0.f, 0.f};

    int b_off[V];
#pragma unroll
    for (int v = 0; v < V; ++v) b_off[v] = (vrow[v] * PW + vcol[v]) * S + 4 * kq;
    int row_blk[MT], row_co[MT];
#pragma unroll
    for (int m = 0; m < MT; ++m) { int r = m * 16 + n; row_blk[m] = r / COUT; row_co[m] = r % COUT; }

    constexpr int NG = 9 * (CIN / 16);
    auto sweep = [&](auto Pc, auto Mc, const float* buf, auto&& extra) __attribute__((always_inline)) {
        constexpr int P = decltype(Pc)::value, TM = decltype(Mc)::value;
        int a_off[MT];
#pragma unroll
        for (int m = 0; m < MT; ++m) {
            int b = row_blk[m];
            int kd = (b < 3) ? ((P - b + 3) % 3) : 0;
            a_off[m] = (kq * NROWS + kd * COUT + row_co[m]) * 4;
        }
        f32x4 bv[2][V], av[2][MT];
        auto load_grp = [&](int g, f32x4 (&b)[V], f32x4 (&aop)[MT]) __attribute__((always_inline)) {
            const int tap = g / (CIN / 16), s = g % (CIN / 16);
            const int kh = tap / 3, kw = tap % 3;
#pragma unroll
            for (int v = 0; v < V; ++v) b[v] = *(const f32x4*)(buf + b_off[v] + (kh * PW + kw) * S + 16 * s);
#pragma unroll
            for (int m = 0; m < MT; ++m) aop[m] = *(const f32x4*)(wl + a_off[m] + (tap * CQ + 4 * s) * WROW);
        };
        load_grp(0, bv[0], av[0]);
#pragma unroll
        for (int g = 0; g < NG; ++g) {
            if (g + 1 < NG) load_grp(g + 1, bv[(g + 1) & 1], av[(g + 1) & 1]);
            __builtin_amdgcn_sched_barrier(0);
            extra(g);
#pragma unroll
            for (int j = 0; j < 4; ++j)
#pragma unroll
                for (int m = 0; m < MT; ++m)
#pragma unroll
                    for (int v = 0; v < V; ++v)
                        if ((TM >> m) & 1) acc[m][v] = __builtin_amdgcn_mfma_f32_16x16x4f32(av[g & 1][m][j], bv[g & 1][v][j], acc[m][v], 0, 0, 0);
            __builtin_amdgcn_sched_barrier(0);
        }
    };

    int yoff[V];
    const int yplane_bytes = a.H * a.W * a.cout_total * 4;
    auto retire = [&](auto Pc, int o) __attribute__((always_inline)) {
        constexpr int P = decltype(Pc)::value;
        constexpr int B = (P + 1) % 3;
        constexpr int mt = (B * COUT) / 16;
        constexpr int row0 = (B * COUT) % 16;
        const bool plane_ok = (o >= d0) && (o < d1);
        const bool mine = (4 * kq >= row0) && (4 * kq < row0 + COUT);
        const int co = 4 * kq - row0;
#pragma unroll
        for (int v = 0; v < V; ++v) {
            if (mine) {
                if (plane_ok) {
                    f32x4 r = acc[mt][v];
                    u32x4_t u = {__float_as_uint(r[0]), __float_as_uint(r[1]), __float_as_uint(r[2]), __float_as_uint(r[3])};
                    __builtin_amdgcn_raw_buffer_store_b128(u, yrsrc, yoff[v] + co * 4, o * yplane_bytes, 0);
                    if (yoff[v] >= 0) {
#pragma unroll
                        for (int k = 0; k < 4; ++k) { st_s[k] += r[k]; st_q[k] += r[k] * r[k]; }
                    }
                }
                acc[mt][v] = (f32x4){0.f, 0.f, 0.f, 0.f};
            }
        }
    };
#pragma unroll
    for (int v = 0; v < V; ++v) {
        const int h = h0 + vrow[v], w = w0 + vcol[v];
        yoff[v] = (h < a.H && w < a.W) ? ((h * a.W + w) * a.cout_total + co_base) * 4 : OOB;
    }

    constexpr int COUT2 = 32;
    float wS2[FUSE2 ? 3 : 1][FUSE2 ? 9 : 1][2];
    f32x4 cur2[2][2], prv2[2][2];
    int s2b[3];
    float st2_s[2][4], st2_q[2][4];
    int fin_od = -1;
    const int Ho2 = a.H / 2, Wo2 = a.W / 2;
    if (FUSE2) {
#pragma unroll
        for (int kd = 0; kd < 3; ++kd)
#pragma unroll
            for (int tap = 0; tap < 9; ++tap)
#pragma unroll
                for (int rt = 0; rt < 2; ++rt)
                    wS2[kd][tap][rt] = fa.w2[((size_t)(kd * 9 + tap) * CIN + 4 * wave + kq) * COUT2 + 16 * rt + n];
#pragma unroll
        for (int kw = 0; kw < 3; ++kw) s2b[kw] = ((2 * (n >> 3) + 1) * PW + 2 * (n & 7) + kw + 1) * S + 4 * wave + kq;
#pragma unroll
        for (int rt = 0; rt < 2; ++rt) {
#pragma unroll
            for (int ct = 0; ct < 2; ++ct) { cur2[rt][ct] = (f32x4){0.f, 0.f, 0.f, 0.f}; prv2[rt][ct] = cur2[rt][ct]; }
#pragma unroll
            for (int k = 0; k < 4; ++k) { st2_s[rt][k] = 0.f; st2_q[rt][k] = 0.f; }
        }
    }
    auto s2_sweep = [&](auto Ec, const float* buf) __attribute__((always_inline)) {
        constexpr int MODE = decltype(Ec)::value;
        float b2[3][2];
        auto ld = [&](int tap, float (&b)[2]) __attribute__((always_inline)) {
            const int kh = tap / 3, kw = tap % 3;
#pragma unroll
            for (int ct = 0; ct < 2; ++ct) b[ct] = buf[s2b[kw] + (4 * ct + kh) * PW * S];
        };
        ld(0, b2[0]); ld(1, b2[1]);
#pragma unroll
        for (int tap = 0; tap < 9; ++tap) {
            if (tap + 2 < 9) ld(tap + 2, b2[(tap + 2) % 3]);
#pragma unroll
            for (int rt = 0; rt < 2; ++rt)
#pragma unroll
                for (int ct = 0; ct < 2; ++ct) {
                    const float bval = b2[tap % 3][ct];
                    if (MODE) {
                        if (MODE == 1) cur2[rt][ct] = __builtin_amdgcn_mfma_f32_16x16x4f32(wS2[0][tap][rt], bval, cur2[rt][ct], 0, 0, 0);
                        prv2[rt][ct] = __builtin_amdgcn_mfma_f32_16x16x4f32(wS2[FUSE2 ? 2 : 0][tap][rt], bval, prv2[rt][ct], 0, 0, 0);
                    } else {
                        cur2[rt][ct] = __builtin_amdgcn_mfma_f32_16x16x4f32(wS2[FUSE2 ? 1 : 0][tap][rt], bval, cur2[rt][ct], 0, 0, 0);
                    }
                }
            __builtin_amdgcn_sched_barrier(0);
        }
    };
    auto s2_finish = [&]() __attribute__((always_inline)) {
        if (fin_od >= 0 && wave == 0) {
#pragma unroll
            for (int rt = 0; rt < 2; ++rt)
#pragma unroll
                for (int ct = 0; ct < 2; ++ct) {
                    f32x4 r = prv2[rt][ct];
#pragma unroll
                    for (int w = 0; w < 3; ++w) {
                        const f32x4 p = *(const f32x4*)(red2 + (((w * 2 + rt) * 2 + ct) * 64 + lane) * 4);
                        r[0] += p[0]; r[1] += p[1]; r[2] += p[2]; r[3] += p[3];
                    }
                    const int oh = h0 / 2 + 2 * ct + (n >> 3), ow = w0 / 2 + (n & 7);
                    if (oh < Ho2 && ow < Wo2) {
                        float* dst = fa.y2 + ((((size_t)fin_od * Ho2 + oh) * Wo2) + ow) * COUT2 + 16 * rt + 4 * kq;
                        *(float4*)dst = make_float4(r[0], r[1], r[2], r[3]);
#pragma unroll
                        for (int k = 0; k < 4; ++k) { st2_s[rt][k] += r[k]; st2_q[rt][k] += r[k] * r[k]; }
                    }
                }
        }
        fin_od = -1;
    };

    const bool trim_first = fa.full_sweeps == 0 || (fa.full_sweeps == 2 && d0 == 0);
    const bool trim_last = fa.full_sweeps == 0 || (fa.full_sweeps == 2 && d1 == a.D);
    const int t_first = trim_first && d0 == 0 ? 1 : 0;
    {
        float* buf = slab + (t_first & 1) * SLAB_FLOATS;
#pragma unroll
        for (int i = 0; i < NIT; ++i) load_piece(i, d0 - 1 + t_first);
#pragma unroll
        for (int i = 0; i < NIT; ++i) stage_piece(i, d0 - 1 + t_first, buf);
#pragma unroll
        for (int i = 0; i < NIT; ++i) load_piece(i, d0 + t_first);
        __syncthreads();
    }

    auto plane = [&](auto Pc, int t) __attribute__((always_inline)) {
        const int q = d0 - 1 + t;
        float* cur = slab + (t & 1) * SLAB_FLOATS;
        float* nxt = slab + ((t + 1) & 1) * SLAB_FLOATS;
        auto extra = [&](int g) __attribute__((always_inline)) {
#pragma unroll
            for (int i = 0; i < NIT; ++i) {
                if ((i * (NG / 2)) / NIT == g) stage_piece(i, q + 1, nxt);
                if (NG / 2 + (i * (NG - NG / 2)) / NIT == g) load_piece(i, q + 2);
            }
        };
        if (FUSE2) s2_finish();
        sweep(Pc, std::integral_constant<int, (1 << MT) - 1>{}, cur, extra);
        if (FUSE2 && q >= d0) {
            const bool in_vol = q < a.D;
            if (q & 1) {
                if (in_vol) s2_sweep(std::false_type{}, cur);
            } else {
#pragma unroll
                for (int rt = 0; rt < 2; ++rt)
#pragma unroll
                    for (int ct = 0; ct < 2; ++ct) { prv2[rt][ct] = cur2[rt][ct]; cur2[rt][ct] = (f32x4){0.f, 0.f, 0.f, 0.f}; }
                if (in_vol) s2_sweep(std::true_type{}, cur);
                const int od_prev = q / 2 - 1;
                if (2 * od_prev >= d0) {
                    if (wave > 0) {
#pragma unroll
                        for (int rt = 0; rt < 2; ++rt)
#pragma unroll
                            for (int ct = 0; ct < 2; ++ct)
                                *(f32x4*)(red2 + ((((wave - 1) * 2 + rt) * 2 + ct) * 64 + lane) * 4) = prv2[rt][ct];
                    }
                    fin_od = od_prev;
                }
            }
        }
        retire(Pc, q - 1);
        __syncthreads();
    };
    auto first_plane = [&]() __attribute__((always_inline)) {
        const int q = d0 - 1;
        float* nxt = slab + SLAB_FLOATS;
        auto extra = [&](int g) __attribute__((always_inline)) {
#pragma unroll
            for (int i = 0; i < NIT; ++i) {
                if ((i * (NG / 2)) / NIT == g) stage_piece(i, q + 1, nxt);
                if (NG / 2 + (i * (NG - NG / 2)) / NIT == g) load_piece(i, q + 2);
            }
        };
        sweep(std::integral_constant<int, 0>{}, std::integral_constant<int, 1>{}, slab, extra);
        retire(std::integral_constant<int, 0>{}, q - 1);
        __syncthreads();
    };
    auto last_plane = [&](auto Pc) __attribute__((always_inline)) {
        constexpr int P = decltype(Pc)::value;
        constexpr int mt = (((P + 1) % 3) * COUT) / 16;
        const int q = d1;
        const float* cur = slab + ((T - 1) & 1) * SLAB_FLOATS;
        const bool in_vol = q < a.D;
        if (FUSE2) s2_finish();
        if (in_vol) sweep(Pc, std::integral_constant<int, 1 << mt>{}, cur, [](int) {});
        if (FUSE2) {
#pragma unroll
            for (int rt = 0; rt < 2; ++rt)
#pragma unroll
                for (int ct = 0; ct < 2; ++ct) { prv2[rt][ct] = cur2[rt][ct]; cur2[rt][ct] = (f32x4){0.f, 0.f, 0.f, 0.f}; }
            if (in_vol) s2_sweep(std::integral_constant<int, 2>{}, cur);
            const int od_prev = q / 2 - 1;
            if (2 * od_prev >= d0) {
                if (wave > 0) {
#pragma unroll
                    for (int rt = 0; rt < 2; ++rt)
#pragma unroll
                        for (int ct = 0; ct < 2; ++ct)
                            *(f32x4*)(red2 + ((((wave - 1) * 2 + rt) * 2 + ct) * 64 + lane) * 4) = prv2[rt][ct];
                }
                fin_od = od_prev;
            }
        }
        retire(Pc, q - 1);
        __syncthreads();
    };
    const int t_lo = trim_first ? 1 : 0, t_hi = trim_last ? T - 1 : T;
    if (trim_first && d0 > 0) first_plane();
    for (int t = 0; t < t_hi; t += 3) {
        if (t >= t_lo) plane(std::integral_constant<int, 0>{}, t);
        if (t + 1 < t_hi) plane(std::integral_constant<int, 1>{}, t + 1);
        if (t + 2 < t_hi) plane(std::integral_constant<int, 2>{}, t + 2);
    }
    if (trim_last) {
        const int pl = (T - 1) % 3;
        if (pl == 0) last_plane(std::integral_constant<int, 0>{});
        else if (pl == 1) last_plane(std::integral_constant<int, 1>{});
        else last_plane(std::integral_constant<int, 2>{});
    }

    if (FUSE2) {
        s2_finish();
        if (fa.stats2 && wave == 0) {
            double* s2p = fa.stats2 + (size_t)((blockIdx.x + gridDim.x * blockIdx.z) % (fa.slots2 > 1 ? fa.slots2 : 1)) * 2 * COUT2;
#pragma unroll
            for (int rt = 0; rt < 2; ++rt)
#pragma unroll
                for (int k = 0; k < 4; ++k) {
                    float sv = st2_s[rt][k], qv = st2_q[rt][k];
#pragma unroll
                    for (int o = 8; o > 0; o >>= 1) { sv += __shfl_xor(sv, o, 64); qv += __shfl_xor(qv, o, 64); }
                    if (n == 0) {
                        atomicAdd(&s2p[16 * rt + 4 * kq + k], (double)sv);
                        atomicAdd(&s2p[COUT2 + 16 * rt + 4 * kq + k], (double)qv);
                    }
                }
        }
        __syncthreads();
    }

    if (a.stats) stats_commit<COUT>(st_s, st_q, COUT == 8, slab, conv_stats_row(a), a.cout_total, co_base);
}

template <int CIN, int COUT, int TH, int TWG = CONV_TW, int CR = 1>
int launch_s1(const ConvArgs& a0, int Cout, hipStream_t st, int slots = 256) {
    ConvArgs a = a0;
    if ((long long)a.D * a.H * a.W * (CIN > Cout ? CIN : Cout) * 4 >= (1LL << 31)) return MVS_E_SHAPE;
    const int tiles = ((a.H + TH - 1) / TH) * ((a.W + TWG - 1) / TWG);
    const int groups = Cout / COUT;
    a.planes_per_wg = conv_pick_planes(a.D, (long long)tiles * groups, 2, slots);
    if (const int hk = mvs_hook(MVS_HOOK_S1_PLANES)) a.planes_per_wg = hk < a.D ? hk : a.D;
    const Fuse2Args fa = {nullptr, nullptr, nullptr, 0, (mvs_hook(MVS_HOOK_CONV_FULL_SWEEPS) >> 2) & 3};
    dim3 grid(tiles, groups, (a.D + a.planes_per_wg - 1) / a.planes_per_wg);
    size_t smem = (size_t)S1Geom<CIN, COUT, TH, TWG>::LDS_BYTES;
    static bool attr_done = false;
    if (!attr_done) {
        hipError_t e;
        if ((e = hipFuncSetAttribute((const void*)conv3d_s1_kernel<CIN, COUT, TH, true, TWG, CR>,
                                     hipFuncAttributeMaxDynamicSharedMemorySize, (int)smem)) != hipSuccess) return (int)e;
        if ((e = hipFuncSetAttribute((const void*)conv3d_s1_kernel<CIN, COUT, TH, false, TWG, CR>,
                                     hipFuncAttributeMaxDynamicSharedMemorySize, (int)smem)) != hipSuccess) return (int)e;
        attr_done = true;
    }
    if (a.x2) conv3d_s1_kernel<CIN, COUT, TH, true, TWG, CR><<<grid, 256, smem, st>>>(a, fa);
    else conv3d_s1_kernel<CIN, COUT, TH, false, TWG, CR><<<grid, 256, smem, st>>>(a, fa);
    return (int)hipGetLastError();
}

int launch_s1_fuse2(const ConvArgs& a0, const Fuse2Args& fa, hipStream_t st) {
    ConvArgs a = a0;
    if ((a.D & 1) || (a.H & 1) || (a.W & 1) || a.x2 || a.cout_total != 16) return MVS_E_SHAPE;
    if ((long long)a.D * a.H * a.W * 16 * 4 >= (1LL << 31)) return MVS_E_SHAPE;
    const int tiles = ((a.H + 7) / 8) * ((a.W + CONV_TW - 1) / CONV_TW);
    int best = 2; long long best_cost = 1LL << 60;
    for (int dr = 2; dr <= a.D; dr += 2) {
        const long long wgs = (long long)tiles * ((a.D + dr - 1) / dr);
        const long long cost = ((wgs + 255) / 256) * (dr + 3);
        if (cost < best_cost) { best_cost = cost; best = dr; }
    }
    a.planes_per_wg = best;
    if (const int hk = mvs_hook(MVS_HOOK_FUSE2_PLANES)) a.planes_per_wg = hk < a.D ? hk : a.D;
    dim3 grid(tiles, 1, (a.D + a.planes_per_wg - 1) / a.planes_per_wg);
    const size_t smem = (size_t)S1Geom<16, 16, 8>::LDS_BYTES + FUSE2_RED_FLOATS * sizeof(float);
    static bool attr_done = false;
    if (!attr_done) {
        hipError_t e = hipFuncSetAttribute((const void*)conv3d_s1_kernel<16, 16, 8, false, CONV_TW, 1, true>,
                                           hipFuncAttributeMaxDynamicSharedMemorySize, (int)smem);
        if (e != hipSuccess) return (int)e;
        attr_done = true;
    }
    conv3d_s1_kernel<16, 16, 8, false, CONV_TW, 1, true><<<grid, 256, smem, st>>>(a, fa);
    return (int)hipGetLastError();
}

}

int mvs_conv3d_dispatch(ConvArgs& a, int Cin, int Cout, int stride, hipStream_t st) {
    if (stride == 1) {
        if (Cout == 1) return mvs_conv3d_out_launch(a, Cin, st);
        if (Cin == 1) return mvs_conv3d_in1_launch(a, Cout, st);
        if (Cin == 8) return mvs_conv3d_k8_launch(a, Cout, st);
        if (a.wprep_bf && mvs_conv3d_bf16x3_supported(Cin, Cout)) return mvs_conv3d_s1_bf16x3(a, Cin, Cout, st);
        if (mvs_conv3d_os_covers(0, Cin, Cout)) return mvs_conv3d_os_launch(a, 0, Cin, Cout, st);
        if (Cin == 32 && Cout == 8 && !a.x2) {
            int rc = mvs_conv3d_c8_launch(a, st);
            if (rc != MVS_E_SHAPE) return rc;
        }
        if (Cin == 32 && Cout == 8) return launch_s1<32, 8, 8>(a, Cout, st);
        if (Cin == 16 && Cout % 16 == 0) return launch_s1<16, 16, 8>(a, Cout, st);
        if (Cin == 32 && Cout % 16 == 0 && a.W % 16 != 0 && a.W % 8 == 0) return launch_s1<32, 16, 8, 8, 2>(a, Cout, st);
        if (Cin == 32 && Cout % 16 == 0) return launch_s1<32, 16, 8>(a, Cout, st);
        if (Cin == 64 && Cout % 8 == 0 && a.W % 16 != 0 && a.W % 4 == 0 && a.H % 16 == 0) return launch_s1<64, 8, 16, 4, 4>(a, Cout, st);
        if (Cin == 64 && Cout % 8 == 0) return launch_s1<64, 8, 4>(a, Cout, st);
        if (Cin == 16 && Cout == 8) return launch_s1<16, 8, 8>(a, Cout, st);
        return MVS_E_SHAPE;
    }
    auto pad_before = [](int n) { int o = (n + 1) / 2; int t = (o - 1) * 2 + 3 - n; return t < 0 ? 0 : t / 2; };
    a.pd = pad_before(a.D); a.ph = pad_before(a.H); a.pw = pad_before(a.W);
    if (mvs_conv3d_os_covers(1, Cin, Cout)) return mvs_conv3d_os_launch(a, 1, Cin, Cout, st);
    return mvs_conv3d_s2_mfma(a, Cin, Cout, st);
}

int mvs_conv3d_s1_fuse2_launch(const ConvArgs& a, const float* w2, float* y2, double* stats2, hipStream_t st) {
    if (mvs_hook(MVS_HOOK_CONV_NO_FUSE2)) return MVS_E_SHAPE;
    return launch_s1_fuse2(a, Fuse2Args{w2, y2, stats2, a.stats_slots, (mvs_hook(MVS_HOOK_CONV_FULL_SWEEPS) >> 2) & 3}, st);
}

namespace {
__global__ void weight_layout_kernel(const float* __restrict__ w, int kind, int Cin, int Cout, int G,
                                     float* __restrict__ out) {
    const int total = 27 * Cin * Cout;
    int i = blockIdx.x * blockDim.x + threadIdx.x;
    if (i >= total) return;
    const int per_group = 27 * Cin * G;
    const int g = i / per_group;
    int r = i - g * per_group;
    const int j = r & 3; r >>= 2;
    const int CQ = Cin / 4;
    if (kind == 2) {
        const int co = r % G; r /= G;
        const int ciq = r % CQ, tap = r / CQ;
        out[i] = w[((size_t)tap * Cout + g * G + co) * Cin + ciq * 4 + j];
    } else {
        const int rows = 3 * G;
        const int row = r % rows; r /= rows;
        const int ciq = r % CQ, tap = r / CQ;
        const int kd = row / G, co = row - kd * G;
        out[i] = w[((size_t)(kd * 9 + tap) * Cin + ciq * 4 + j) * Cout + g * G + co];
    }
}
}

int mvs_conv_weight_layout(const float* w, int kind, int Cin, int Cout, float* out, hipStream_t st) {
    if (mvs_conv3d_os_covers(kind, Cin, Cout)) return mvs_conv3d_os_weight_layout(w, kind, Cin, Cout, out, st);
    const int G = conv_coutg(kind, Cin, Cout);
    if (G == 0 || (Cin % 4)) return MVS_E_SHAPE;
    const int total = 27 * Cin * Cout;
    weight_layout_kernel<<<mvs_cdiv(total, 256), 256, 0, st>>>(w, kind, Cin, Cout, G, out);
    return (int)hipGetLastError();
}
```

mvsnet_amd/csrc/conv_common.h:

```cpp
#pragma once
#include "common.h"
#include <type_traits>

typedef float f32x4 __attribute__((ext_vector_type(4)));

struct BnSrc {
    const double* stats;
    const float* gamma; const float* beta;
    double count; float eps; int C;
    int nslot;
};

__device__ __forceinline__ void bn_affine_finish(double s1, double s2, double inv_count, float gamma, float beta, float eps,
                                                 float& scale, float& shift) {
    const double mean = s1 * inv_count;
    double var = s2 * inv_count - mean * mean;
    if (var < 0.0) var = 0.0;
    const float inv = gamma * __builtin_amdgcn_rsqf((float)var + eps);
    scale = inv;
    shift = beta - (float)mean * inv;
}

constexpr int MVS_BN_SLOTS_MAX = 8;
struct BnSum1 { double s1, s2; float g, b; bool mine; };
__device__ __forceinline__ BnSum1 bn_sum1(const BnSrc& b, int t0) {
    BnSum1 r = {0.0, 0.0, 0.f, 0.f, false};
    const int c = (int)threadIdx.x - t0;
    if (c < 0 || c >= b.C) return r;
    double p1[MVS_BN_SLOTS_MAX], p2[MVS_BN_SLOTS_MAX];
#pragma unroll
    for (int sl = 0; sl < MVS_BN_SLOTS_MAX; ++sl) {
        const int row = sl < b.nslot ? sl : 0;
        p1[sl] = b.stats[row * 2 * b.C + c]; p2[sl] = b.stats[row * 2 * b.C + b.C + c];
    }
    r.s1 = p1[0]; r.s2 = p2[0];
#pragma unroll
    for (int sl = 1; sl < MVS_BN_SLOTS_MAX; ++sl)
        if (sl < b.nslot) { r.s1 += p1[sl]; r.s2 += p2[sl]; }
    r.g = b.gamma[c]; r.b = b.beta[c]; r.mine = true;
    return r;
}
__device__ __forceinline__ void bn_fold_store(const BnSrc& b, const BnSum1& r, int t0, float* tab) {
    if (!r.mine) return;
    const int c = (int)threadIdx.x - t0;
    float s, t;
    bn_affine_finish(r.s1, r.s2, 1.0 / b.count, r.g, r.b, b.eps, s, t);
    tab[c] = s; tab[b.C + c] = t;
}
__device__ __forceinline__ void bn_fold_to_lds(const BnSrc& b, int t0, float* tab) { bn_fold_store(b, bn_sum1(b, t0), t0, tab); }
__device__ __forceinline__ void bn_affine4_lds(const float* tab, int C, int c0, float4& sc, float4& sh) {
    sc = *(const float4*)(tab + c0);
    sh = *(const float4*)(tab + C + c0);
}
__device__ __forceinline__ void bn_affine4_wg(const BnSrc& b1, bool use1, const BnSrc& b2, bool use2, float* tab, int c0,
                                              float4& sc, float4& sh, float4& sc2, float4& sh2) {
    const bool f1 = use1 && b1.stats, f2 = use2 && b2.stats;
    if (!f1 && !f2) return;
    float* tab2 = tab + (f1 ? 2 * b1.C : 0);
    if (f1) bn_fold_to_lds(b1, 0, tab);
    if (f2) bn_fold_to_lds(b2, 128, tab2);
    __syncthreads();
    if (f1) bn_affine4_lds(tab, b1.C, c0, sc, sh);
    if (f2) bn_affine4_lds(tab2, b2.C, c0, sc2, sh2);
}

struct ConvArgs {
    const float* x = nullptr; const float* xs = nullptr; const float* xb = nullptr;
    const float* x2 = nullptr; const float* x2s = nullptr; const float* x2b = nullptr;
    const float* w = nullptr;
    float* y = nullptr;
    double* stats = nullptr;
    int D = 0, H = 0, W = 0, cout_total = 0, planes_per_wg = 0;
    int pd = 0, ph = 0, pw = 0;
    BnSrc bn = {}, bn2 = {};
    const float* wprep = nullptr;
    const unsigned short* wprep_bf = nullptr;
    int stats_slots = 0;
};
static inline ConvArgs conv_args(const float* x, const float* w, float* y, double* stats, int D, int H, int W, int cout_total) {
    ConvArgs a;
    a.x = x; a.w = w; a.y = y; a.stats = stats; a.D = D; a.H = H; a.W = W; a.cout_total = cout_total;
    return a;
}

__device__ __forceinline__ double* conv_stats_row(const ConvArgs& a) {
    const int slots = a.stats_slots > 1 ? a.stats_slots : 1;
    return a.stats + (size_t)((blockIdx.x + gridDim.x * blockIdx.z) % slots) * 2 * a.cout_total;
}

constexpr int CONV_TW = 16;

template <int CIN> struct SlabGeom { static constexpr int S = CIN + 8; };

__device__ __forceinline__ float4 bn_relu4(float4 v, float4 s, float4 b, bool aff) {
    if (aff) {
        v.x = relu(v.x * s.x + b.x); v.y = relu(v.y * s.y + b.y);
        v.z = relu(v.z * s.z + b.z); v.w = relu(v.w * s.w + b.w);
    }
    return v;
}

template <int COUT>
__device__ __forceinline__ void stats_commit(const float (&st_s)[4], const float (&st_q)[4],
                                             bool fold32, float* red_raw, double* stats,
                                             int cout_total, int co_base) {
    float (*red)[2][16] = reinterpret_cast<float (*)[2][16]>(red_raw);
    const int tid = threadIdx.x, lane = tid & 63, wave = tid >> 6;
    const int n = lane & 15, kq = lane >> 4;
    float s[4], q[4];
#pragma unroll
    for (int k = 0; k < 4; ++k) {
        float sv = st_s[k], qv = st_q[k];
#pragma unroll
        for (int o = 8; o > 0; o >>= 1) { sv += __shfl_xor(sv, o, 64); qv += __shfl_xor(qv, o, 64); }
        if (fold32) { sv += __shfl_xor(sv, 32, 64); qv += __shfl_xor(qv, 32, 64); }
        s[k] = sv; q[k] = qv;
    }
    constexpr int ngrp = COUT / 4;
    if (n == 0 && kq < ngrp) {
#pragma unroll
        for (int k = 0; k < 4; ++k) { red[wave][0][4 * kq + k] = s[k]; red[wave][1][4 * kq + k] = q[k]; }
    }
    __syncthreads();
    if (tid < 2 * COUT) {
        int k = tid / COUT, c = tid - k * COUT;
        double t = (double)red[0][k][c] + (double)red[1][k][c] + (double)red[2][k][c] + (double)red[3][k][c];
        atomicAdd(&stats[(size_t)k * cout_total + co_base + c], t);
    }
}

static inline int conv_pick_planes(int D, long long wgs_per_chunk, int halo, int slots = 256) {
    int best = D;
    long long best_cost = 1LL << 60;
    for (int dr = 1; dr <= D; ++dr) {
        long long chunks = (D + dr - 1) / dr;
        long long wgs = wgs_per_chunk * chunks;
        long long rounds = (wgs + slots - 1) / slots;
        long long cost = rounds * (dr + halo + 1);
        if (cost < best_cost) { best_cost = cost; best = dr; }
    }
    return best;
}

static inline int conv_coutg(int kind, int Cin, int Cout) {
    if (kind == 0) {
        if (Cin == 32 && Cout == 8) return 8;
        if (Cin == 16 && Cout % 16 == 0) return 16;
        if (Cin == 32 && Cout % 16 == 0) return 16;
        if (Cin == 64 && Cout % 8 == 0) return 8;
        if (Cin == 16 && Cout == 8) return 8;
        return 0;
    }
    if (kind == 1) return (Cout % 16 == 0 && (Cin == 32 || Cin == 16)) ? 16 : 0;
    if (Cin == 16 && Cout == 8) return 8;
    if (Cin == 32 && Cout % 16 == 0) return 16;
    if (Cin == 64 && Cout % 8 == 0) return 8;
    if (Cin == 16 && Cout % 16 == 0) return 16;
    return 0;
}

__device__ __forceinline__ void copy_weights_to_lds(float* wl, const float* src, int w_floats) {
    const float4* s4 = reinterpret_cast<const float4*>(src);
    float4* d4 = reinterpret_cast<float4*>(wl);
    const int n4 = w_floats / 4;
    for (int i0 = threadIdx.x; i0 < n4; i0 += 8 * 256) {
        float4 t[8];
#pragma unroll
        for (int k = 0; k < 8; ++k) { const int i = i0 + 256 * k; t[k] = i < n4 ? s4[i] : make_float4(0.f, 0.f, 0.f, 0.f); }
#pragma unroll
        for (int k = 0; k < 8; ++k) { const int i = i0 + 256 * k; if (i < n4) d4[i] = t[k]; }
    }
}
__device__ __forceinline__ void load_prepared_weights(float* wl, const float* wprep, int w_floats) {
    copy_weights_to_lds(wl, wprep + (size_t)blockIdx.y * w_floats, w_floats);
}

int mvs_conv3d_dispatch(ConvArgs& a, int Cin, int Cout, int stride, hipStream_t st);
int mvs_conv3d_s1_fuse2_launch(const ConvArgs& a, const float* w2, float* y2, double* stats2, hipStream_t st);
int mvs_conv_weight_layout(const float* w, int kind, int Cin, int Cout, float* out, hipStream_t st);
int mvs_conv3d_scalar(const float* x, const float* xs, const float* xb, const float* x2, const float* x2s, const float* x2b,
                      const float* w, int D, int H, int W, int Cin, int Cout, int stride, float* y, double* stats, hipStream_t st);
int mvs_deconv3d_scalar(const float* x, const float* xs, const float* xb, const float* x2, const float* x2s, const float* x2b,
                        const float* w, int D, int H, int W, int Cin, int Cout, float* y, double* stats, hipStream_t st);
int mvs_homography_transforms_zero(const float* cams, int view_num, int depth_num, float depth_start, float depth_interval,
                                   float depth_end, int inverse_depth, float* transforms, double* zero, int zero_n, hipStream_t st);
bool mvs_stream_set_side(hipStream_t caller, hipStream_t* side, hipEvent_t* fork, hipEvent_t* join);
int mvs_conv3d_s2_mfma(const ConvArgs& a, int Cin, int Cout, hipStream_t st);
int mvs_deconv3d_mfma_launch(const ConvArgs& a, int Cin, int Cout, hipStream_t st);
int mvs_conv3d_out_launch(const ConvArgs& a, int Cin, hipStream_t st);
int mvs_conv3d_in1_launch(const ConvArgs& a, int Cout, hipStream_t st);
int mvs_conv3d_k8_launch(const ConvArgs& a, int Cout, hipStream_t st);
int mvs_wgrad_c1_plan(int D, int H, int W, int CB, int* rows, int* planes_per_wg);
int mvs_wgrad_c1_launch(const float* big, const float* small, int D, int H, int W, int CB, float* partial, hipStream_t st);
int mvs_deconv3d_c8_launch(const ConvArgs& a, int Cin, int Cout, hipStream_t st);
int mvs_conv3d_c8_launch(const ConvArgs& a, hipStream_t st);
int mvs_conv3d_c8_s2_launch(const ConvArgs& a, const float* w2, float* y2, double* stats2, hipStream_t st,
                            int slots1 = 1, int slots2 = 1, const float* wprep_wino = nullptr);
constexpr int MVS_CONV_WINO_FLOATS = 3 * 4 * 32 * 3 * 8;
int mvs_conv_wino_weight_layout(const float* w, float* out, hipStream_t st);
int mvs_conv3d_c8_wino_s2_launch(const ConvArgs& a, const float* wprep_wino, const float* w2, float* y2, double* stats2,
                                 hipStream_t st, int slots1, int slots2);
bool mvs_conv3d_os_covers(int kind, int Cin, int Cout);
int mvs_conv3d_os_weight_layout(const float* w, int kind, int Cin, int Cout, float* out, hipStream_t st);
int mvs_conv3d_os_launch(const ConvArgs& a, int kind, int Cin, int Cout, hipStream_t st);
int mvs_conv3d_os_filler_blocks(int D, int H, int W);
int mvs_conv3d_os_filled_launch(const ConvArgs& a, int kind, int Cin, int Cout, const ConvArgs& b, int b_first, int b_count,
                                hipStream_t st);
bool mvs_conv3d_bf16x3_supported(int Cin, int Cout);
int mvs_conv3d_s1_bf16x3(const ConvArgs& a, int Cin, int Cout, hipStream_t st);
int mvs_conv_weight_split(const float* w, int Cin, int Cout, unsigned short* out, hipStream_t st);
```

mvsnet_amd/csrc/library.hip:

```cpp
#include "profile.h"

extern "C" int mvs_abi_version(void) { return MVS_ABI_VERSION; }

extern "C" const char* mvs_error_string(int code) {
    if (code == 0) return "success";
    if (code == MVS_E_BADARG) return "mvsnet_hip: bad argument (null pointer or non-positive size)";
    if (code == MVS_E_SHAPE) return "mvsnet_hip: shape not supported by this kernel";
    if (code == MVS_E_WORKSPACE) return "mvsnet_hip: workspace too small";
    if (code == MVS_E_NO_SLOT) return "mvsnet_hip: all 16 stream sets of mvs_gru_prepare are in use (mvs_gru_release frees one); the sweep still runs, on the caller's stream alone";
    if (code == MVS_E_NOT_PREPARED) return "mvsnet_hip: no side streams for this caller stream (call mvs_gru_prepare outside hipGraph capture first)";
    if (code > 0) return hipGetErrorString((hipError_t)code);
    return "mvsnet_hip: unknown error";
}

static int g_conv_impl = MVS_CONV_IMPL_AUTO;
extern "C" int mvs_set_conv_impl(int impl) {
    if (impl < MVS_CONV_IMPL_AUTO || impl > MVS_CONV_IMPL_BF16X3) return MVS_E_BADARG;
    g_conv_impl = impl;
    return 0;
}
extern "C" int mvs_get_conv_impl(void) { return g_conv_impl; }

#ifndef MVS_PAIR_DIRECT_DEFAULT
#define MVS_PAIR_DIRECT_DEFAULT 0
#endif
#ifndef MVS_PAIR_WAVES4_DEFAULT
#define MVS_PAIR_WAVES4_DEFAULT 0
#endif
std::atomic<int> mvs_hooks[MVS_HOOK_COUNT] = {{-1}, {0}, {0}, {0}, {0}, {128}, {1}, {0}, {0}, {0}, {0}, {0}, {0}, {0}, {0}, {0}, {0}, {MVS_PAIR_DIRECT_DEFAULT},
                                              {MVS_PAIR_WAVES4_DEFAULT}};
extern "C" int mvs_set_test_hook(int id, int value) {
    bool ok = false;
    switch (id) {
        case MVS_HOOK_CV_TILE_ROWS_LOG2: ok = value >= -1 && value <= 3; break;
        case MVS_HOOK_CONV_NO_SPAN: case MVS_HOOK_CONV_NO_FUSE2: case MVS_HOOK_GRU_ONE_STREAM: case MVS_HOOK_UNET_PERSISTENT:
        case MVS_HOOK_REGNET_SIDE_BRANCH: case MVS_HOOK_PAIR_DIRECT: case MVS_HOOK_PAIR_WAVES4:
            ok = value == 0 || value == 1; break;
        case MVS_HOOK_CONV_FULL_SWEEPS: ok = value >= 0 && value < 16 && (value & 3) < 3 && (value >> 2) < 3; break;
        case MVS_HOOK_UNET_GRID: ok = value >= 0 && value <= 65536; break;
        case MVS_HOOK_FUSE2_PLANES: case MVS_HOOK_PAIR_PLANES: ok = value >= 0 && value <= 65536 && (value & 1) == 0; break;
        case MVS_HOOK_S2_PLANES: case MVS_HOOK_OUT_PLANES: case MVS_HOOK_S1_PLANES: ok = value >= 0 && value <= 65536; break;
        case MVS_HOOK_SPAN_FORCE: ok = value == 0 || ((value >> 8) >= 1 && (value >> 8) <= 8 && (value & 255) >= (value >> 8) && (value & 255) <= 16); break;
        case MVS_HOOK_BN_SLOTS: case MVS_HOOK_PAIR_SLOTS: ok = value >= 0 && value <= 8; break;
        case MVS_HOOK_GRU_PRODUCER_THREADS: ok = value == 64 || value == 128 || value == 192 || value == 256; break;
        default: break;
    }
    if (!ok) return MVS_E_BADARG;
    mvs_hooks[id].store(value, std::memory_order_relaxed);
    return 0;
}
extern "C" int mvs_get_test_hook(int id) {
    if (id < 0 || id >= MVS_HOOK_COUNT) return MVS_E_BADARG;
    return mvs_hooks[id].load(std::memory_order_relaxed);
}

EventSlots<64, 2> mvs_prof_dominant;
EventSlots<32, 22> mvs_prof_layers;
EventSlots<32, 4> mvs_prof_stages;

extern "C" int mvs_profile_dominant(int enable) { mvs_prof_dominant.enable(enable != 0); return 0; }
extern "C" int mvs_profile_dominant_ms(double* avg_ms, int* count) {
    MVS_CHECK_ARG(avg_ms && count);
    return mvs_prof_dominant.read(avg_ms, 1, 2, count);
}
extern "C" int mvs_profile_layers(int enable) { mvs_prof_layers.enable(enable != 0); return 0; }
extern "C" int mvs_profile_layers_ms(double* avg_ms11, int* count) {
    MVS_CHECK_ARG(avg_ms11 && count);
    return mvs_prof_layers.read(avg_ms11, 11, 2, count);
}
extern "C" int mvs_profile_stages(int enable) { mvs_prof_stages.enable(enable != 0); return 0; }
extern "C" int mvs_profile_stages_ms(double* avg_ms3, int* count) {
    MVS_CHECK_ARG(avg_ms3 && count);
    return mvs_prof_stages.read(avg_ms3, 3, 1, count);
}
```

mvsnet_amd/csrc/regnet.hip:

```cpp
#include "conv_common.h"
#include "profile.h"
#include <initializer_list>

extern "C" int mvs_conv3d_f32(const float* x, const float* xs, const float* xb, const float* x2,
                              const float* x2s, const float* x2b, const float* w, int D, int H,
                              int W, int Cin, int Cout, int stride, float* y, double* stats,
                              void* stream) {
    MVS_CHECK_ARG(x && w && y && D > 0 && H > 0 && W > 0 && Cin > 0 && Cout > 0);
    MVS_CHECK_ARG((xs == nullptr) == (xb == nullptr) && (x2s == nullptr) == (x2b == nullptr));
    MVS_CHECK_ARG(stride == 1 || stride == 2);
    hipStream_t st = mvs_stream(stream);
    const int impl = mvs_get_conv_impl();
    if (impl != MVS_CONV_IMPL_SCALAR) {
        ConvArgs a = conv_args(x, w, y, stats, D, H, W, Cout);
        a.xs = xs; a.xb = xb; a.x2 = x2; a.x2s = x2s; a.x2b = x2b;
        int rc = mvs_conv3d_dispatch(a, Cin, Cout, stride, st);
        if (rc != MVS_E_SHAPE || impl == MVS_CONV_IMPL_MFMA) return rc;
    }
    return mvs_conv3d_scalar(x, xs, xb, x2, x2s, x2b, w, D, H, W, Cin, Cout, stride, y, stats, st);
}

extern "C" int mvs_deconv3d_f32(const float* x, const float* xs, const float* xb, const float* x2,
                                const float* x2s, const float* x2b, const float* w, int D, int H,
                                int W, int Cin, int Cout, float* y, double* stats, void* stream) {
    MVS_CHECK_ARG(x && w && y && D > 0 && H > 0 && W > 0 && Cin > 0 && Cout > 0);
    MVS_CHECK_ARG((xs == nullptr) == (xb == nullptr) && (x2s == nullptr) == (x2b == nullptr));
    hipStream_t st = mvs_stream(stream);
    const int impl = mvs_get_conv_impl();
    if (impl != MVS_CONV_IMPL_SCALAR) {
        ConvArgs a = conv_args(x, w, y, stats, D, H, W, Cout);
        a.xs = xs; a.xb = xb; a.x2 = x2; a.x2s = x2s; a.x2b = x2b;
        int rc = mvs_deconv3d_mfma_launch(a, Cin, Cout, st);
        if (rc != MVS_E_SHAPE || impl == MVS_CONV_IMPL_MFMA) return rc;
    }
    return mvs_deconv3d_scalar(x, xs, xb, x2, x2s, x2b, w, D, H, W, Cin, Cout, y, stats, st);
}

extern "C" int mvs_conv3d_pair_f32(const float* x, const float* w1, const float* w2, int D, int H, int W,
                                   int Cin, int Cout1, int Cout2, float* y1, double* stats1,
                                   float* y2, double* stats2, void* stream) {
    MVS_CHECK_ARG(x && w1 && w2 && y1 && y2 && D > 0 && H > 0 && W > 0);
    if (Cin != 32 || Cout1 != 8 || Cout2 != 16 || mvs_get_conv_impl() == MVS_CONV_IMPL_SCALAR) return MVS_E_SHAPE;
    return mvs_conv3d_c8_s2_launch(conv_args(x, w1, y1, stats1, D, H, W, Cout1), w2, y2, stats2, mvs_stream(stream));
}


constexpr int FILL_3_0 = 250, FILL_3_1 = 500;

extern "C" int mvs_regnet_filler_shares(int* permille3) {
    MVS_CHECK_ARG(permille3);
    permille3[0] = FILL_3_0; permille3[1] = FILL_3_1; permille3[2] = 1000 - FILL_3_0 - FILL_3_1;
    return 0;
}

namespace {

constexpr int N_LAYERS = 11, N_BN = 10;
enum { L10, L20, L30, L01, L11, L21, L31, L40, L50, L60, L62 };
enum { S1 = 0, S2 = 1, UP = 2 };
constexpr int COST = 0, ONE = 0;
struct LayerRow {
    int kind;
    int level;
    int ci, co;
    int p1, p2;
};
constexpr LayerRow NET[N_LAYERS] = {
     {S2, 0, COST, 2, -1, -1},
     {S2, 1, 2, 4, L10, -1},
     {S2, 2, 4, 8, L20, -1},
     {S1, 0, COST, 1, -1, -1},
     {S1, 1, 2, 2, L10, -1},
     {S1, 2, 4, 4, L20, -1},
     {S1, 3, 8, 8, L30, -1},
     {UP, 3, 8, 4, L31, -1},
     {UP, 2, 4, 2, L40, L21},
     {UP, 1, 2, 1, L50, L11},
     {S1, 0, 1, ONE, L60, L01},
};
constexpr int out_level(int i) { return NET[i].level + (NET[i].kind == S2) - (NET[i].kind == UP); }
constexpr int widest() { int m = 0; for (const LayerRow& r : NET) m = r.co > m ? r.co : m; return m; }
constexpr int CMAX = widest();

size_t stats_doubles(int b) { return (size_t)N_BN * MVS_BN_SLOTS_MAX * 2 * CMAX * b; }

struct Net {
    int ci[N_LAYERS], co[N_LAYERS];
    size_t woff[N_LAYERS], wtotal;
    bool ok[N_LAYERS], bf[N_LAYERS];
};
Net net_of(int cin, int b) {
    Net n;
    size_t off = 0;
    for (int i = 0; i < N_LAYERS; ++i) {
        const int kind = NET[i].kind, ci = NET[i].ci == COST ? cin : NET[i].ci * b, co = NET[i].co == ONE ? 1 : NET[i].co * b;
        n.ci[i] = ci; n.co[i] = co; n.woff[i] = off;
        n.ok[i] = (i != L62) && (ci % 4 == 0) && conv_coutg(kind, ci, co) != 0;
        n.bf[i] = n.ok[i] && kind == S1 && mvs_conv3d_bf16x3_supported(ci, co);
        off += (size_t)27 * ci * co;
    }
    n.wtotal = off;
    return n;
}

struct RegnetWs {
    float* y[N_BN];
    float* scale[N_BN];
    float* shift[N_BN];
    double* stats;
    size_t bytes;
};

size_t align256(size_t b) { return (b + 255) & ~(size_t)255; }

size_t wino_floats(const Net& n) { return (n.ci[L01] == 32 && n.co[L01] == 8) ? (size_t)MVS_CONV_WINO_FLOATS : 0; }

RegnetWs carve(char* base, int D, int H, int W, int b) {
    const size_t v0 = (size_t)D * H * W;
    size_t off = 0;
    RegnetWs w;
    for (int i = 0; i < N_BN; ++i) {
        w.y[i] = (float*)(base ? base + off : nullptr);
        off += align256((v0 >> (3 * out_level(i))) * NET[i].co * b * sizeof(float));
    }
    for (int i = 0; i < N_BN; ++i) {
        w.scale[i] = (float*)(base ? base + off : nullptr); off += align256(CMAX * b * sizeof(float));
        w.shift[i] = (float*)(base ? base + off : nullptr); off += align256(CMAX * b * sizeof(float));
    }
    w.stats = (double*)(base ? base + off : nullptr);
    off += align256(stats_doubles(b) * sizeof(double));
    w.bytes = off;
    return w;
}

}

extern "C" size_t mvs_regnet_workspace_bytes(int D, int H, int W, int cin, int base) {
    if (D <= 0 || H <= 0 || W <= 0 || cin <= 0 || base <= 0) return 0;
    return carve(nullptr, D, H, W, base).bytes;
}

extern "C" size_t mvs_regnet_prepared_floats(int cin, int base) {
    if (cin <= 0 || base <= 0) return 0;
    const Net n = net_of(cin, base);
    return 2 * n.wtotal + wino_floats(n);
}

extern "C" int mvs_regnet_prepare_f32(const float* const* weights, int cin, int base, float* prepared,
                                      void* stream) {
    MVS_CHECK_ARG(weights && prepared && cin > 0 && base > 0);
    const Net n = net_of(cin, base);
    for (int i = 0; i < N_LAYERS; ++i) {
        if (!n.ok[i]) continue;
        int rc = mvs_conv_weight_layout(weights[i], NET[i].kind, n.ci[i], n.co[i], prepared + n.woff[i], mvs_stream(stream));
        if (rc) return rc;
        if (n.bf[i]) {
            rc = mvs_conv_weight_split(weights[i], n.ci[i], n.co[i],
                                       reinterpret_cast<unsigned short*>(prepared + n.wtotal + n.woff[i]), mvs_stream(stream));
            if (rc) return rc;
        }
    }
    if (wino_floats(n)) return mvs_conv_wino_weight_layout(weights[L01], prepared + 2 * n.wtotal, mvs_stream(stream));
    return 0;
}

namespace {

__global__ void bn_fold_rows_kernel(double* stats, int nslot, int n) {
    for (int j = threadIdx.x; j < n; j += blockDim.x) {
        double t = stats[j];
        for (int r = 1; r < nslot; ++r) { t += stats[(size_t)r * n + j]; stats[(size_t)r * n + j] = 0.0; }
        stats[j] = t;
    }
}

constexpr int BN_SLOTS = 8;
constexpr int PAIR_SLOTS = 2;
static_assert(BN_SLOTS <= MVS_BN_SLOTS_MAX && PAIR_SLOTS <= MVS_BN_SLOTS_MAX, "rows beyond the workspace's slab");
static_assert(MVS_BN_SLOTS_MAX == 8, "mvs_set_test_hook admits 1..8 rows");
int bn_slots() { const int hk = mvs_hook(MVS_HOOK_BN_SLOTS); return hk ? hk : BN_SLOTS; }
int pair_slots() { const int hk = mvs_hook(MVS_HOOK_PAIR_SLOTS); return hk ? hk : PAIR_SLOTS; }

struct Run {
    const float* cost; int batch, D, H, W, b;
    const float* const* weights; const float* prepared; const float* const* gammas; const float* const* betas;
    float eps; float* reg; hipStream_t hs;
    int impl;
    Net net;
    RegnetWs ws;
    size_t ws_floats1;
    bool all_mfma;
    int SL;
    int PS;
    int lp;
    bool pair_done = false;
    bool finalised[N_BN] = {};

    double* st(int i) const { return ws.stats + (size_t)i * MVS_BN_SLOTS_MAX * 2 * CMAX * b; }
    int nslot_of(int i) const { return (pair_done && (i == L01 || i == L10)) ? PS : SL; }
    BnSrc bn_of(int i) const {
        if (i < 0) return BnSrc{nullptr, nullptr, nullptr, 1.0, eps, 0, 1};
        return BnSrc{st(i), gammas[i], betas[i], count(i), eps, net.co[i], nslot_of(i)};
    }
    double count(int i) const { return ((double)batch * D * H * W) / (double)(1 << (3 * out_level(i))); }
    const float* wprep(int i) const { return (prepared && net.ok[i]) ? prepared + net.woff[i] : nullptr; }
    const float* wprep_wino() const { return (prepared && wino_floats(net)) ? prepared + 2 * net.wtotal : nullptr; }
    int mark(int l, int k, hipStream_t s) const { return mvs_prof_layers.mark(lp, 2 * l + k, s); }
};

ConvArgs layer_args(const Run& r, int bi, int out) {
    const LayerRow& row = NET[out];
    const size_t wo = (size_t)bi * r.ws_floats1;
    const size_t v0 = (size_t)r.D * r.H * r.W;
    ConvArgs a = conv_args(row.p1 >= 0 ? r.ws.y[row.p1] + wo : r.cost + (size_t)bi * v0 * r.net.ci[out], r.weights[out],
                           out == L62 ? r.reg + (size_t)bi * v0 : r.ws.y[out] + wo, out == L62 ? nullptr : r.st(out),
                           r.D >> row.level, r.H >> row.level, r.W >> row.level, r.net.co[out]);
    a.x2 = row.p2 >= 0 ? r.ws.y[row.p2] + wo : nullptr;
    a.bn = r.bn_of(row.p1); a.bn2 = r.bn_of(row.p2);
    a.wprep = r.wprep(out);
    if (r.prepared && r.impl == MVS_CONV_IMPL_BF16X3 && r.net.bf[out] && (!r.all_mfma || out == L01))
        a.wprep_bf = reinterpret_cast<const unsigned short*>(r.prepared + r.net.wtotal + r.net.woff[out]);
    a.stats_slots = r.SL;
    return a;
}

int ensure_final(Run& r, int i) {
    if (i < 0 || r.finalised[i]) return 0;
    r.finalised[i] = true;
    if (r.nslot_of(i) > 1) {
        bn_fold_rows_kernel<<<1, 256, 0, r.hs>>>(r.st(i), r.nslot_of(i), 2 * r.net.co[i]);
        hipError_t e = hipGetLastError();
        if (e != hipSuccess) return (int)e;
    }
    return mvs_bn_finalize_f32(r.st(i), r.net.co[i], r.count(i), r.gammas[i], r.betas[i], r.eps, r.ws.scale[i], r.ws.shift[i], r.hs);
}

int layer_one(Run& r, int bi, int out, hipStream_t s) {
    const LayerRow& row = NET[out];
    ConvArgs a = layer_args(r, bi, out);
    const int ci = r.net.ci[out], co = r.net.co[out];
    if (r.impl != MVS_CONV_IMPL_SCALAR) {
        int rc = row.kind == UP ? mvs_deconv3d_mfma_launch(a, ci, co, s) : mvs_conv3d_dispatch(a, ci, co, row.kind == S2 ? 2 : 1, s);
        if (rc != MVS_E_SHAPE || r.impl != MVS_CONV_IMPL_AUTO) return rc;
    }
    int rc;
    if ((rc = ensure_final(r, row.p1)) || (rc = ensure_final(r, row.p2))) return rc;
    const float* s1 = row.p1 >= 0 ? r.ws.scale[row.p1] : nullptr; const float* t1 = row.p1 >= 0 ? r.ws.shift[row.p1] : nullptr;
    const float* s2 = row.p2 >= 0 ? r.ws.scale[row.p2] : nullptr; const float* t2 = row.p2 >= 0 ? r.ws.shift[row.p2] : nullptr;
    return row.kind == UP ? mvs_deconv3d_scalar(a.x, s1, t1, a.x2, s2, t2, a.w, a.D, a.H, a.W, ci, co, a.y, a.stats, s)
                          : mvs_conv3d_scalar(a.x, s1, t1, a.x2, s2, t2, a.w, a.D, a.H, a.W, ci, co, row.kind == S2 ? 2 : 1, a.y, a.stats, s);
}

int layer(Run& r, int out, hipStream_t s) {
    int rc = r.mark(out, 0, s);
    for (int bi = 0; bi < r.batch && !rc; ++bi) rc = layer_one(r, bi, out, s);
    return rc ? rc : r.mark(out, 1, s);
}

constexpr int APART = -1000;

int or_apart(Run& r, int rc, std::initializer_list<int> layers) {
    if (rc != APART) return rc;
    for (int l : layers) if ((rc = layer(r, l, r.hs))) return rc;
    return 0;
}

int fused_pair(Run& r) {
    if (!((r.impl == MVS_CONV_IMPL_AUTO || r.impl == MVS_CONV_IMPL_MFMA) && r.net.ci[L01] == 32 && r.b == 8)) return APART;
    const int slot = mvs_prof_dominant.claim();
    int rc;
    if ((rc = mvs_prof_dominant.mark(slot, 0, r.hs)) || (rc = r.mark(L01, 0, r.hs))) return rc;
    for (int bi = 0; bi < r.batch; ++bi) {
        const size_t wo = (size_t)bi * r.ws_floats1;
        ConvArgs a = conv_args(r.cost + (size_t)bi * r.D * r.H * r.W * r.net.ci[L01], r.weights[L01], r.ws.y[L01] + wo, r.st(L01),
                               r.D, r.H, r.W, r.net.co[L01]);
        a.wprep = r.wprep(L01);
        rc = mvs_conv3d_c8_s2_launch(a, r.weights[L10], r.ws.y[L10] + wo, r.st(L10), r.hs, r.PS, r.PS, r.wprep_wino());
        if (rc) return rc == MVS_E_SHAPE ? APART : rc;
    }
    if ((rc = r.mark(L01, 1, r.hs)) || (rc = mvs_prof_dominant.mark(slot, 1, r.hs))) return rc;
    mvs_prof_dominant.commit(slot);
    r.pair_done = true;
    return 0;
}

int fuse2(Run& r) {
    const int D1 = r.D >> 1, H1 = r.H >> 1, W1 = r.W >> 1;
    if (!r.all_mfma || (D1 & 1) || (H1 & 1) || (W1 & 1)) return APART;
    int rc = r.mark(L11, 0, r.hs);
    for (int bi = 0; bi < r.batch && !rc; ++bi) {
        const size_t wo = (size_t)bi * r.ws_floats1;
        ConvArgs a = conv_args(r.ws.y[L10] + wo, r.weights[L11], r.ws.y[L11] + wo, r.st(L11), D1, H1, W1, r.net.co[L11]);
        a.bn = r.bn_of(L10); a.wprep = r.wprep(L11); a.stats_slots = r.SL;
        rc = mvs_conv3d_s1_fuse2_launch(a, r.weights[L20], r.ws.y[L20] + wo, r.st(L20), r.hs);
    }
    if (rc) return rc == MVS_E_SHAPE ? APART : rc;
    return r.mark(L11, 1, r.hs);
}

struct SideBranch {
    hipStream_t hs = nullptr, side = nullptr;
    hipEvent_t ev_fork = nullptr, ev_join = nullptr;
    enum { NONE, FORKED, BRANCH_RECORDED } state = NONE;
    int fork() {
        hipError_t e = hipEventRecord(ev_fork, hs);
        if (e == hipSuccess) e = hipStreamWaitEvent(side, ev_fork, 0);
        if (e == hipSuccess) state = FORKED;
        return (int)e;
    }
    int branch_end() {
        const hipError_t e = hipEventRecord(ev_join, side);
        if (e == hipSuccess) state = BRANCH_RECORDED;
        return (int)e;
    }
    int join() {
        if (state == NONE) return 0;
        hipError_t e = state == FORKED ? hipEventRecord(ev_join, side) : hipSuccess;
        if (e == hipSuccess) e = hipStreamWaitEvent(hs, ev_join, 0);
        state = NONE;
        return (int)e;
    }
    ~SideBranch() { join(); }
};
int side_branch(Run& r, SideBranch& sb) {
    int rc;
    if ((rc = sb.fork()) || (rc = layer(r, L11, sb.side)) || (rc = sb.branch_end())) return rc;
    return layer(r, L20, r.hs);
}

int filled_chain(Run& r) {
    if (!(r.all_mfma && r.prepared && r.net.ok[L21] && r.net.ok[L30] && r.net.ok[L31] && r.net.ok[L40])) return APART;
    const int nfill = mvs_conv3d_os_filler_blocks(r.D >> 2, r.H >> 2, r.W >> 2);
    const int f0 = (nfill * FILL_3_0 / 1000) & ~7, f1 = (nfill * FILL_3_1 / 1000) & ~7;
    const int chain[3] = {L30, L31, L40}, first[3] = {0, f0, f0 + f1}, count[3] = {f0, f1, nfill - f0 - f1};
    for (int k = 0; k < 3; ++k) {
        const int out = chain[k];
        int rc = r.mark(out, 0, r.hs);
        for (int bi = 0; bi < r.batch && !rc; ++bi)
            rc = mvs_conv3d_os_filled_launch(layer_args(r, bi, out), NET[out].kind, r.net.ci[out], r.net.co[out],
                                             layer_args(r, bi, L21), first[k], count[k], r.hs);
        if (!rc) rc = r.mark(out, 1, r.hs);
        if (rc) return (rc == MVS_E_SHAPE && k == 0) ? APART : rc;
    }
    return 0;
}

int regnet_run(const float* cost, int batch, int D, int H, int W, int cin, int base,
               const float* const* weights, const float* prepared, const float* const* gammas,
               const float* const* betas, float eps, void* workspace, size_t workspace_bytes,
               float* reg, void* stream, bool stats_zeroed = false) {
    MVS_CHECK_ARG(cost && weights && gammas && betas && workspace && reg);
    MVS_CHECK_ARG(batch > 0 && D > 0 && H > 0 && W > 0 && cin > 0 && base > 0);
    if ((D % 8) || (H % 8) || (W % 8)) return MVS_E_SHAPE;
    const RegnetWs ws = carve((char*)workspace, D, H, W, base);
    if (workspace_bytes < ws.bytes * (size_t)batch) return MVS_E_WORKSPACE;
    int rc;
    if (!stats_zeroed && (rc = mvs_zero_f64(ws.stats, stats_doubles(base), stream))) return rc;
    const int impl = mvs_get_conv_impl();
    const bool all_mfma = impl != MVS_CONV_IMPL_SCALAR && cin == 32 && base == 8 && (long long)D * H * W * cin * 4 < (1LL << 31);
    Run r{cost, batch, D, H, W, base, weights, prepared, gammas, betas, eps, reg, mvs_stream(stream), impl,
          net_of(cin, base), ws, ws.bytes / sizeof(float), all_mfma, all_mfma ? bn_slots() : 1, pair_slots(), mvs_prof_layers.claim()};
    mvs_prof_layers.commit(r.lp);

    SideBranch sb;
    bool side = false;
    if (mvs_hook(MVS_HOOK_REGNET_SIDE_BRANCH) && all_mfma && batch == 1 && r.lp < 0) {
        hipStreamCaptureStatus cs = hipStreamCaptureStatusNone;
        const bool capturing = hipStreamIsCapturing(r.hs, &cs) == hipSuccess && cs != hipStreamCaptureStatusNone;
        sb.hs = r.hs;
        side = !capturing && mvs_stream_set_side(r.hs, &sb.side, &sb.ev_fork, &sb.ev_join);
    }
    if ((rc = or_apart(r, fused_pair(r), {L10, L01}))) return rc;
    if ((rc = or_apart(r, side ? side_branch(r, sb) : fuse2(r), {L11, L20}))) return rc;
    if ((rc = or_apart(r, filled_chain(r), {L21, L30, L31, L40}))) return rc;
    if ((rc = layer(r, L50, r.hs))) return rc;
    if ((rc = sb.join())) return rc;
    if ((rc = layer(r, L60, r.hs))) return rc;
    return layer(r, L62, r.hs);
}

}

extern "C" int mvs_regnet_us0_f32(const float* cost, int D, int H, int W, int cin, int base,
                                  const float* const* weights, const float* const* gammas,
                                  const float* const* betas, float eps, void* workspace,
                                  size_t workspace_bytes, float* reg, void* stream) {
    return regnet_run(cost, 1, D, H, W, cin, base, weights, nullptr, gammas, betas, eps, workspace,
                      workspace_bytes, reg, stream);
}

extern "C" int mvs_regnet_us0_prepared_f32(const float* cost, int D, int H, int W, int cin, int base,
                                           const float* const* weights, const float* prepared,
                                           const float* const* gammas, const float* const* betas,
                                           float eps, void* workspace, size_t workspace_bytes,
                                           float* reg, void* stream) {
    MVS_CHECK_ARG(prepared);
    return regnet_run(cost, 1, D, H, W, cin, base, weights, prepared, gammas, betas, eps, workspace,
                      workspace_bytes, reg, stream);
}

extern "C" int mvs_regnet_us0_batch_f32(const float* cost, int batch, int D, int H, int W, int cin, int base,
                                        const float* const* weights, const float* prepared,
                                        const float* const* gammas, const float* const* betas,
                                        float eps, void* workspace, size_t workspace_bytes,
                                        float* reg, void* stream) {
    return regnet_run(cost, batch, D, H, W, cin, base, weights, prepared, gammas, betas, eps, workspace,
                      workspace_bytes, reg, stream);
}

extern "C" int mvs_depth_from_features_f32(const float* features, const float* cams, int view_num, int depth_num,
                                           int H, int W, int C, int base, float depth_start, float depth_interval,
                                           float depth_end, int inverse_depth, int variant,
                                           const float* const* weights, const float* prepared,
                                           const float* const* gammas, const float* const* betas, float eps,
                                           float* transforms, float* cost, void* workspace, size_t workspace_bytes,
                                           float* reg, float* depth, float* prob, void* stream) {
    MVS_CHECK_ARG(features && cams && weights && gammas && betas && transforms && cost && workspace && reg && depth && prob);
    MVS_CHECK_ARG(view_num >= 2 && depth_num >= 1 && H > 0 && W > 0 && C > 0 && base > 0);
    if ((depth_num % 8) || (H % 8) || (W % 8)) return MVS_E_SHAPE;
    RegnetWs ws = carve((char*)workspace, depth_num, H, W, base);
    if (workspace_bytes < ws.bytes) return MVS_E_WORKSPACE;
    int rc;
    const int sp = mvs_prof_stages.claim();
    mvs_prof_stages.commit(sp);
    auto mark = [&](int k) { return mvs_prof_stages.mark(sp, k, mvs_stream(stream)); };
    if ((rc = mark(0))) return rc;
    if ((rc = mvs_homography_transforms_zero(cams, view_num, depth_num, depth_start, depth_interval, depth_end, inverse_depth,
                                             transforms, ws.stats, (int)stats_doubles(base), mvs_stream(stream)))) return rc;
    if ((rc = mvs_cost_volume_f32(features, features + (size_t)H * W * C, transforms, view_num, depth_num, 0, depth_num,
                                  H, W, C, variant, 0, 0, cost, stream))) return rc;
    if ((rc = mark(1))) return rc;
    if ((rc = regnet_run(cost, 1, depth_num, H, W, C, base, weights, prepared, gammas, betas, eps, workspace,
                         workspace_bytes, reg, stream, true))) return rc;
    if ((rc = mark(2))) return rc;
    if ((rc = mvs_softargmin_prob_f32(reg, depth_num, H, W, depth_start, depth_interval, inverse_depth, depth, prob, stream))) return rc;
    return mark(3);
}
```

Measured before the change: 1141 depth maps/s.

## Add Winograd F(2,3) kernel for fused stride-1 16->16 conv with stride-2 follow-up

Adds a new kernel that computes the 16-channel stride-1 3D conv (L11) using a 1D Winograd F(2,3) transform along W, fused with the following stride-2 conv (L20). It uses weights pre-transformed during the prepare step. The fuse2 path now routes to this kernel by default, with a hook to fall back to the direct MFMA kernel. The intent is to cut the MFMA count for L11; the cost is more LDS use, transform arithmetic, and slightly different float rounding.

```diff
diff --git a/include/mvsnet_hip.h b/include/mvsnet_hip.h
--- a/include/mvsnet_hip.h
+++ b/include/mvsnet_hip.h
@@ -45,7 +45,8 @@
 #define MVS_HOOK_SPAN_FORCE           16
 #define MVS_HOOK_PAIR_DIRECT          17
 #define MVS_HOOK_PAIR_WAVES4          18
-#define MVS_HOOK_COUNT                19
+#define MVS_HOOK_FUSE2_DIRECT         19
+#define MVS_HOOK_COUNT                20
 int mvs_set_test_hook(int id, int value);
 int mvs_get_test_hook(int id);
 
@@ -74,6 +75,10 @@
 int mvs_conv3d_pair_f32(const float* x, const float* w1, const float* w2, int D, int H, int W,
                         int Cin, int Cout1, int Cout2, float* y1, double* stats1,
                         float* y2, double* stats2, void* stream);
+
+int mvs_conv3d_fuse2_f32(const float* x, const float* xs, const float* xb, const float* w1, const float* w2,
+                         int D, int H, int W, int Cin, int Cout1, int Cout2, float* y1, double* stats1,
+                         float* y2, double* stats2, void* stream);
 
 int mvs_bn_finalize_f32(const double* stats, int C, double count, const float* gamma,
                         const float* beta, float eps, float* scale, float* shift, void* stream);
diff --git a/mvsnet_amd/_lib.py b/mvsnet_amd/_lib.py
--- a/mvsnet_amd/_lib.py
+++ b/mvsnet_amd/_lib.py
@@ -26,6 +26,7 @@
     "mvs_conv3d_f32": (_i, [_p] * 7 + [_i] * 6 + [_p, _p, _p]),
     "mvs_deconv3d_f32": (_i, [_p] * 7 + [_i] * 5 + [_p, _p, _p]),
     "mvs_conv3d_pair_f32": (_i, [_p] * 3 + [_i] * 6 + [_p] * 5),
+    "mvs_conv3d_fuse2_f32": (_i, [_p] * 5 + [_i] * 6 + [_p] * 5),
     "mvs_gn_stat_slots": (_i, []),
     "mvs_conv2d_prepared_floats": (_sz, [_i, _i, _i, _i]),
     "mvs_conv2d_prepare_f32": (_i, [_p, _i, _i, _i, _i, _p, _p]),
@@ -156,11 +157,11 @@
 HOOKS = {"cv_tile_rows_log2": 0, "conv_no_span": 1, "conv_no_fuse2": 2, "s2_planes": 3, "gru_one_stream": 4,
          "gru_producer_threads": 5, "unet_persistent": 6, "unet_grid": 7, "fuse2_planes": 8, "regnet_side_branch": 9,
          "out_planes": 10, "bn_slots": 11, "pair_slots": 12, "conv_full_sweeps": 13, "pair_planes": 14, "s1_planes": 15,
-         "span_force": 16, "pair_direct": 17, "pair_waves4": 18}
+         "span_force": 16, "pair_direct": 17, "pair_waves4": 18, "fuse2_direct": 19}
 HOOK_DEFAULTS = {"cv_tile_rows_log2": -1, "conv_no_span": 0, "conv_no_fuse2": 0, "s2_planes": 0, "gru_one_stream": 0,
                  "gru_producer_threads": 128, "unet_persistent": 1, "unet_grid": 0, "fuse2_planes": 0, "regnet_side_branch": 0,
                  "out_planes": 0, "bn_slots": 0, "pair_slots": 0, "conv_full_sweeps": 0, "pair_planes": 0, "s1_planes": 0,
-                 "span_force": 0, "pair_direct": 0, "pair_waves4": 0}
+                 "span_force": 0, "pair_direct": 0, "pair_waves4": 0, "fuse2_direct": 0}
 
 _lib = None
 
diff --git a/mvsnet_amd/build.py b/mvsnet_amd/build.py
--- a/mvsnet_amd/build.py
+++ b/mvsnet_amd/build.py
@@ -9,7 +9,7 @@
 CSRC = os.path.join(HERE, "csrc")
 LIB_PATH = os.path.join(HERE, "libmvsnet_hip.so")
 SOURCES = ["homography.hip", "cost_volume.hip", "conv3d_scalar.hip", "conv3d_mfma.hip", "conv3d_s2_mfma.hip",
-           "deconv3d_mfma.hip", "deconv3d_c8.hip", "conv3d_os.hip", "conv3d_out.hip", "conv3d_bf16x3.hip", "conv3d_c8.hip", "conv3d_c8_wino.hip",
+           "deconv3d_mfma.hip", "deconv3d_c8.hip", "conv3d_os.hip", "conv3d_out.hip", "conv3d_bf16x3.hip", "conv3d_c8.hip", "conv3d_c8_wino.hip", "conv3d_s1_wino.hip",
            "regnet.hip", "library.hip", "softargmin.hip", "gru.hip", "gru_mfma.hip", "gru_fused.hip", "gru_streams.hip", "gru_sweep.hip", "unet2d.hip", "unet2d_p.hip", "center_images.hip", "multi_tensor.hip",
            "backward.hip", "groupnorm.hip", "optimizer.hip", "conv3d_wgrad.hip", "conv3d_c1.hip", "conv3d_k8.hip", "gru_train.hip", "conv2d_wgrad.hip",
            "fusion.hip", "pointcloud.hip", "render.hip", "view_selection.hip", "tsdf.hip", "raster.hip", "mesh_components.hip", "mesh_simplify.hip", "mesh_sample.hip"]
diff --git a/mvsnet_amd/csrc/conv3d_c8_wino.hip b/mvsnet_amd/csrc/conv3d_c8_wino.hip
--- a/mvsnet_amd/csrc/conv3d_c8_wino.hip
+++ b/mvsnet_amd/csrc/conv3d_c8_wino.hip
@@ -34,12 +34,6 @@
     return (row * PW + pc) * SP + (((slot + 2 * (pc >> 1)) & 7) << 2);
 }
 
-__device__ __forceinline__ float wino_u(float g0, float g1, float g2, int pt) {
-    if (pt == 0) return g0;
-    if (pt == 3) return g2;
-    const double s = (double)g0 + (double)g2;
-    return (float)(0.5 * (pt == 1 ? s + (double)g1 : s - (double)g1));
-}
 __device__ __forceinline__ float wino_weight(const float* __restrict__ w, int i) {
     const int j = i & 3;
     const int r = (i >> 2) % NROWS;
diff --git a/mvsnet_amd/csrc/conv3d_mfma.hip b/mvsnet_amd/csrc/conv3d_mfma.hip
--- a/mvsnet_amd/csrc/conv3d_mfma.hip
+++ b/mvsnet_amd/csrc/conv3d_mfma.hip
@@ -450,7 +450,7 @@
     return (int)hipGetLastError();
 }
 
-int launch_s1_fuse2(const ConvArgs& a0, const Fuse2Args& fa, hipStream_t st) {
+int launch_s1_fuse2(const ConvArgs& a0, const Fuse2Args& fa, const float* wprep_wino, hipStream_t st) {
     ConvArgs a = a0;
     if ((a.D & 1) || (a.H & 1) || (a.W & 1) || a.x2 || a.cout_total != 16) return MVS_E_SHAPE;
     if ((long long)a.D * a.H * a.W * 16 * 4 >= (1LL << 31)) return MVS_E_SHAPE;
@@ -463,6 +463,8 @@
     }
     a.planes_per_wg = best;
     if (const int hk = mvs_hook(MVS_HOOK_FUSE2_PLANES)) a.planes_per_wg = hk < a.D ? hk : a.D;
+    if (!mvs_hook(MVS_HOOK_FUSE2_DIRECT))
+        return mvs_conv3d_s1_wino_fuse2_launch(a, wprep_wino, fa.w2, fa.y2, fa.stats2, fa.full_sweeps, st);
     dim3 grid(tiles, 1, (a.D + a.planes_per_wg - 1) / a.planes_per_wg);
     const size_t smem = (size_t)S1Geom<16, 16, 8>::LDS_BYTES + FUSE2_RED_FLOATS * sizeof(float);
     static bool attr_done = false;
@@ -504,9 +506,9 @@
     return mvs_conv3d_s2_mfma(a, Cin, Cout, st);
 }
 
-int mvs_conv3d_s1_fuse2_launch(const ConvArgs& a, const float* w2, float* y2, double* stats2, hipStream_t st) {
+int mvs_conv3d_s1_fuse2_launch(const ConvArgs& a, const float* w2, float* y2, double* stats2, hipStream_t st, const float* wprep_wino) {
     if (mvs_hook(MVS_HOOK_CONV_NO_FUSE2)) return MVS_E_SHAPE;
-    return launch_s1_fuse2(a, Fuse2Args{w2, y2, stats2, a.stats_slots, (mvs_hook(MVS_HOOK_CONV_FULL_SWEEPS) >> 2) & 3}, st);
+    return launch_s1_fuse2(a, Fuse2Args{w2, y2, stats2, a.stats_slots, (mvs_hook(MVS_HOOK_CONV_FULL_SWEEPS) >> 2) & 3}, wprep_wino, st);
 }
 
 namespace {
diff --git a/mvsnet_amd/csrc/conv3d_s1_wino.hip b/mvsnet_amd/csrc/conv3d_s1_wino.hip
--- /dev/null
+++ b/mvsnet_amd/csrc/conv3d_s1_wino.hip
@@ -0,0 +1,399 @@
+#include "conv_common.h"
+
+namespace {
+
+constexpr int CIN = 16, COUT = 16, COUT2 = 32, CQ = CIN / 4;
+constexpr int TH = 8, TW = CONV_TW;
+constexpr int PW = TW + 2;
+constexpr int RP = PW + 1;
+constexpr int S = SlabGeom<CIN>::S;
+constexpr int ROWF = RP * S;
+constexpr int NPOS = (TH + 2) * PW;
+constexpr int NF4 = NPOS * CQ;
+constexpr int NIT = (NF4 + 255) / 256;
+constexpr int NROWS = 3 * COUT;
+constexpr int WROW = NROWS * 4;
+constexpr int NPT = 4;
+constexpr int NG = 3 * NPT;
+constexpr int W_FLOATS = NG * CQ * WROW;
+constexpr int SLAB_FLOATS = (TH + 2) * ROWF;
+constexpr int RED_FLOATS = 3 * 2 * 2 * 64 * 4;
+constexpr int LDS_FLOATS = W_FLOATS + 2 * SLAB_FLOATS + RED_FLOATS;
+static_assert(W_FLOATS == MVS_CONV_S1_WINO_FLOATS, "the regulariser reserves this many prepared floats");
+static_assert(NF4 >= 256 && 256 % CQ == 0, "staging map");
+
+typedef unsigned int u32x4_t __attribute__((ext_vector_type(4)));
+constexpr int OOB = (int)0x80000000u;
+
+__device__ __forceinline__ float s1_wino_weight(const float* __restrict__ w, int i) {
+    const int j = i & 3;
+    const int r = (i >> 2) % NROWS;
+    const int g = (i >> 2) / NROWS;
+    const int ciq = g % CQ, tap = g / CQ;
+    const int kh = tap >> 2, pt = tap & 3;
+    const int kd = r / COUT, co = r - kd * COUT;
+    const float* p = w + ((size_t)((kd * 3 + kh) * 3) * CIN + ciq * 4 + j) * COUT + co;
+    return wino_u(p[0], p[CIN * COUT], p[2 * CIN * COUT], pt);
+}
+
+__global__ void s1_wino_weight_layout_kernel(const float* __restrict__ w, float* __restrict__ out) {
+    const int i = blockIdx.x * blockDim.x + threadIdx.x;
+    if (i < W_FLOATS) out[i] = s1_wino_weight(w, i);
+}
+
+struct WinoS1Args {
+    const float* wprep;
+    const float* w2;
+    float* y2;
+    double* stats2;
+    int slots2;
+    int full_sweeps;
+};
+
+__global__ void __launch_bounds__(256, 1)
+conv3d_s1_wino_kernel(ConvArgs a, WinoS1Args fa) {
+    extern __shared__ __attribute__((aligned(16))) float smem[];
+    float* wl = smem;
+    float* slab = smem + W_FLOATS;
+    float* red2 = slab + 2 * SLAB_FLOATS;
+
+    const int tid = threadIdx.x;
+    const int lane = tid & 63, wave = __builtin_amdgcn_readfirstlane(tid >> 6);
+    const int n = lane & 15, kq = lane >> 4;
+
+    const int tiles_w = (a.W + TW - 1) / TW;
+    const int bid = xcd_swizzle(blockIdx.x, gridDim.x);
+    const int tile_h = bid / tiles_w, tile_w = bid - tile_h * tiles_w;
+    const int h0 = tile_h * TH, w0 = tile_w * TW;
+    const int d0 = blockIdx.z * a.planes_per_wg;
+    const int d1 = min(d0 + a.planes_per_wg, a.D);
+    const int T = d1 - d0 + 2;
+
+    if (fa.wprep) copy_weights_to_lds(wl, fa.wprep, W_FLOATS);
+    else for (int i = tid; i < W_FLOATS; i += 256) wl[i] = s1_wino_weight(a.w, i);
+
+    const int c4 = tid % CQ;
+    float4 sc = make_float4(1.f, 1.f, 1.f, 1.f), sh = make_float4(0.f, 0.f, 0.f, 0.f);
+    float4 sc2 = sc, sh2 = sh;
+    const bool has_aff = a.xs != nullptr || a.bn.stats != nullptr;
+    if (a.xs) { sc = *(const float4*)(a.xs + 4 * c4); sh = *(const float4*)(a.xb + 4 * c4); }
+    __shared__ __attribute__((aligned(16))) float bn_tab[2 * CIN];
+    bn_affine4_wg(a.bn, !a.xs, a.bn2, false, bn_tab, 4 * c4, sc, sh, sc2, sh2);
+    const float lo = has_aff ? 0.f : -INFINITY;
+
+    float4 pre[NIT];
+    int goff[NIT], loff[NIT];
+#pragma unroll
+    for (int i = 0; i < NIT; ++i) {
+        int f = tid + 256 * i;
+        if (f >= NF4) f -= 256;
+        int pos = f / CQ;
+        int r = pos / PW, c = pos - r * PW;
+        int gh = h0 - 1 + r, gw = w0 - 1 + c;
+        bool inb = gh >= 0 && gh < a.H && gw >= 0 && gw < a.W;
+        goff[i] = inb ? ((gh * a.W + gw) * CIN + 4 * c4) * 4 : OOB;
+        loff[i] = (r * RP + c) * S + 4 * c4;
+    }
+    const int plane_bytes = a.H * a.W * CIN * 4;
+    const auto xrsrc = __builtin_amdgcn_make_buffer_rsrc((void*)a.x, 0, a.D * plane_bytes, 0x00020000);
+    const auto yrsrc = __builtin_amdgcn_make_buffer_rsrc((void*)a.y, 0, a.D * a.H * a.W * COUT * 4, 0x00020000);
+
+    auto load_piece = [&](int i, int q) __attribute__((always_inline)) {
+        const bool plane_ok = (q >= 0) && (q < a.D);
+        u32x4_t v = __builtin_amdgcn_raw_buffer_load_b128(xrsrc, goff[i] | (plane_ok ? 0 : OOB), plane_ok ? q * plane_bytes : 0, 0);
+        pre[i] = make_float4(__uint_as_float(v[0]), __uint_as_float(v[1]), __uint_as_float(v[2]), __uint_as_float(v[3]));
+    };
+    auto stage_piece = [&](int i, int q, float* buf) __attribute__((always_inline)) {
+        const bool ok = (q >= 0) && (q < a.D) && goff[i] >= 0;
+        float4 v = pre[i];
+        v.x = fmaxf(v.x * sc.x + sh.x, lo); v.y = fmaxf(v.y * sc.y + sh.y, lo);
+        v.z = fmaxf(v.z * sc.z + sh.z, lo); v.w = fmaxf(v.w * sc.w + sh.w, lo);
+        v.x = ok ? v.x : 0.f; v.y = ok ? v.y : 0.f; v.z = ok ? v.z : 0.f; v.w = ok ? v.w : 0.f;
+        *(float4*)(buf + loff[i]) = v;
+    };
+    auto staging = [&](int G, int q, float* nxt) __attribute__((always_inline)) {
+#pragma unroll
+        for (int i = 0; i < NIT; ++i) {
+            if (G == 1 + 2 * i) stage_piece(i, q + 1, nxt);
+            if (G == NG / 2 + 1 + 2 * i) load_piece(i, q + 2);
+        }
+    };
+
+    f32x4 acc[NPT][3];
+#pragma unroll
+    for (int p = 0; p < NPT; ++p)
+#pragma unroll
+        for (int m = 0; m < 3; ++m) acc[p][m] = (f32x4){0.f, 0.f, 0.f, 0.f};
+    float st_s[4] = {0.f, 0.f, 0.f, 0.f}, st_q[4] = {0.f, 0.f, 0.f, 0.f};
+
+    const int vr = 2 * wave + (n >> 3), vp = n & 7;
+    const int b_off = (vr * RP + 2 * vp) * S + 4 * kq;
+    const int a_lane = (kq * NROWS + n) * 4;
+
+    auto sweep = [&](auto Pc, auto Mc, const float* buf, auto&& head, auto&& extra) __attribute__((always_inline)) {
+        constexpr int P = decltype(Pc)::value, TM = decltype(Mc)::value;
+        int a_off[3];
+#pragma unroll
+        for (int m = 0; m < 3; ++m) a_off[m] = a_lane + ((P - m + 3) % 3) * COUT * 4;
+        f32x4 av[2][3], raw[4], tb[2][NPT];
+        auto load_a = [&](int G) __attribute__((always_inline)) {
+#pragma unroll
+            for (int m = 0; m < 3; ++m)
+                if ((TM >> m) & 1) av[G & 1][m] = *(const f32x4*)(wl + a_off[m] + G * CQ * WROW);
+        };
+        auto load_raw = [&](int kh, int c) __attribute__((always_inline)) {
+            raw[c] = *(const f32x4*)(buf + b_off + kh * ROWF + c * S);
+        };
+        auto form = [&](int kh, int pt) __attribute__((always_inline)) {
+            tb[kh & 1][pt] = pt == 0 ? raw[0] - raw[2] : pt == 1 ? raw[1] + raw[2] : pt == 2 ? raw[2] - raw[1] : raw[1] - raw[3];
+        };
+        load_a(0);
+#pragma unroll
+        for (int c = 0; c < 4; ++c) load_raw(0, c);
+        __builtin_amdgcn_sched_barrier(0);
+        head();
+        __builtin_amdgcn_sched_barrier(0);
+#pragma unroll
+        for (int pt = 0; pt < NPT; ++pt) form(0, pt);
+#pragma unroll
+        for (int G = 0; G < NG; ++G) {
+            const int kh = G >> 2, pt = G & 3;
+#pragma unroll
+            for (int j = 0; j < 4; ++j) {
+#pragma unroll
+                for (int m = 0; m < 3; ++m)
+                    if ((TM >> m) & 1) acc[pt][m] = __builtin_amdgcn_mfma_f32_16x16x4f32(av[G & 1][m][j], tb[kh & 1][pt][j], acc[pt][m], 0, 0, 0);
+                if (j == 0 && G + 1 < NG) load_a(G + 1);
+                if (j == 1 && kh < 2 && pt < 2) { load_raw(kh + 1, 2 * pt); load_raw(kh + 1, 2 * pt + 1); }
+                if (j == 2 && kh < 2 && pt >= 2) { form(kh + 1, 2 * pt - 4); form(kh + 1, 2 * pt - 3); }
+                if (j == 3) extra(G);
+                __builtin_amdgcn_sched_barrier(0);
+            }
+        }
+    };
+
+    const int yoff = (h0 + vr < a.H && w0 + 2 * vp < a.W) ? (((h0 + vr) * a.W + w0 + 2 * vp) * COUT + 4 * kq) * 4 : OOB;
+    const int yplane_bytes = a.H * a.W * COUT * 4;
+    auto retire = [&](auto Pc, int o) __attribute__((always_inline)) {
+        constexpr int B = (decltype(Pc)::value + 1) % 3;
+        if ((o >= d0) && (o < d1)) {
+            const f32x4 m0 = acc[0][B], m1 = acc[1][B], m2 = acc[2][B], m3 = acc[3][B];
+            f32x4 y[2];
+            y[0] = (m0 + m1) + m2;
+            y[1] = (m1 - m2) - m3;
+#pragma unroll
+            for (int e = 0; e < 2; ++e) {
+                u32x4_t v = {__float_as_uint(y[e][0]), __float_as_uint(y[e][1]), __float_as_uint(y[e][2]), __float_as_uint(y[e][3])};
+                __builtin_amdgcn_raw_buffer_store_b128(v, yrsrc, yoff + e * COUT * 4, o * yplane_bytes, 0);
+                if (yoff >= 0) {
+#pragma unroll
+                    for (int k = 0; k < 4; ++k) { st_s[k] += y[e][k]; st_q[k] = __builtin_fmaf(y[e][k], y[e][k], st_q[k]); }
+                }
+            }
+        }
+#pragma unroll
+        for (int p = 0; p < NPT; ++p) acc[p][B] = (f32x4){0.f, 0.f, 0.f, 0.f};
+    };
+
+    float wS2[3][9][2];
+    f32x4 cur2[2][2], prv2[2][2];
+    int s2b[3];
+    float st2_s[2][4], st2_q[2][4];
+    int fin_od = -1;
+    const int Ho2 = a.H / 2, Wo2 = a.W / 2;
+#pragma unroll
+    for (int kd = 0; kd < 3; ++kd)
+#pragma unroll
+        for (int tap = 0; tap < 9; ++tap)
+#pragma unroll
+            for (int rt = 0; rt < 2; ++rt)
+                wS2[kd][tap][rt] = fa.w2[((size_t)(kd * 9 + tap) * CIN + 4 * wave + kq) * COUT2 + 16 * rt + n];
+#pragma unroll
+    for (int kw = 0; kw < 3; ++kw) s2b[kw] = ((2 * (n >> 3) + 1) * RP + 2 * (n & 7) + kw + 1) * S + 4 * wave + kq;
+#pragma unroll
+    for (int rt = 0; rt < 2; ++rt) {
+#pragma unroll
+        for (int ct = 0; ct < 2; ++ct) { cur2[rt][ct] = (f32x4){0.f, 0.f, 0.f, 0.f}; prv2[rt][ct] = cur2[rt][ct]; }
+#pragma unroll
+        for (int k = 0; k < 4; ++k) { st2_s[rt][k] = 0.f; st2_q[rt][k] = 0.f; }
+    }
+    auto s2_sweep = [&](auto Ec, const float* buf) __attribute__((always_inline)) {
+        constexpr int MODE = decltype(Ec)::value;
+        float b2[3][2];
+        auto ld = [&](int tap, float (&b)[2]) __attribute__((always_inline)) {
+            const int kh = tap / 3, kw = tap % 3;
+#pragma unroll
+            for (int ct = 0; ct < 2; ++ct) b[ct] = buf[s2b[kw] + (4 * ct + kh) * ROWF];
+        };
+        ld(0, b2[0]); ld(1, b2[1]);
+#pragma unroll
+        for (int tap = 0; tap < 9; ++tap) {
+            if (tap + 2 < 9) ld(tap + 2, b2[(tap + 2) % 3]);
+#pragma unroll
+            for (int rt = 0; rt < 2; ++rt)
+#pragma unroll
+                for (int ct = 0; ct < 2; ++ct) {
+                    const float bval = b2[tap % 3][ct];
+                    if (MODE) {
+                        if (MODE == 1) cur2[rt][ct] = __builtin_amdgcn_mfma_f32_16x16x4f32(wS2[0][tap][rt], bval, cur2[rt][ct], 0, 0, 0);
+                        prv2[rt][ct] = __builtin_amdgcn_mfma_f32_16x16x4f32(wS2[2][tap][rt], bval, prv2[rt][ct], 0, 0, 0);
+                    } else {
+                        cur2[rt][ct] = __builtin_amdgcn_mfma_f32_16x16x4f32(wS2[1][tap][rt], bval, cur2[rt][ct], 0, 0, 0);
+                    }
+                }
+            __builtin_amdgcn_sched_barrier(0);
+        }
+    };
+    auto s2_turn = [&]() __attribute__((always_inline)) {
+#pragma unroll
+        for (int rt = 0; rt < 2; ++rt)
+#pragma unroll
+            for (int ct = 0; ct < 2; ++ct) { prv2[rt][ct] = cur2[rt][ct]; cur2[rt][ct] = (f32x4){0.f, 0.f, 0.f, 0.f}; }
+    };
+    auto s2_park = [&](int q) __attribute__((always_inline)) {
+        const int od_prev = q / 2 - 1;
+        if (2 * od_prev >= d0) {
+            if (wave > 0) {
+#pragma unroll
+                for (int rt = 0; rt < 2; ++rt)
+#pragma unroll
+                    for (int ct = 0; ct < 2; ++ct)
+                        *(f32x4*)(red2 + ((((wave - 1) * 2 + rt) * 2 + ct) * 64 + lane) * 4) = prv2[rt][ct];
+            }
+            fin_od = od_prev;
+        }
+    };
+    auto s2_finish = [&]() __attribute__((always_inline)) {
+        if (fin_od >= 0 && wave == 0) {
+#pragma unroll
+            for (int rt = 0; rt < 2; ++rt)
+#pragma unroll
+                for (int ct = 0; ct < 2; ++ct) {
+                    f32x4 r = prv2[rt][ct];
+#pragma unroll
+                    for (int w = 0; w < 3; ++w) {
+                        const f32x4 p = *(const f32x4*)(red2 + (((w * 2 + rt) * 2 + ct) * 64 + lane) * 4);
+                        r[0] += p[0]; r[1] += p[1]; r[2] += p[2]; r[3] += p[3];
+                    }
+                    const int oh = h0 / 2 + 2 * ct + (n >> 3), ow = w0 / 2 + (n & 7);
+                    if (oh < Ho2 && ow < Wo2) {
+                        float* dst = fa.y2 + ((((size_t)fin_od * Ho2 + oh) * Wo2) + ow) * COUT2 + 16 * rt + 4 * kq;
+                        *(float4*)dst = make_float4(r[0], r[1], r[2], r[3]);
+#pragma unroll
+                        for (int k = 0; k < 4; ++k) { st2_s[rt][k] += r[k]; st2_q[rt][k] += r[k] * r[k]; }
+                    }
+                }
+        }
+        fin_od = -1;
+    };
+
+    const bool trim_first = fa.full_sweeps == 0 || (fa.full_sweeps == 2 && d0 == 0);
+    const bool trim_last = fa.full_sweeps == 0 || (fa.full_sweeps == 2 && d1 == a.D);
+    const int t_first = trim_first && d0 == 0 ? 1 : 0;
+    {
+        float* buf = slab + (t_first & 1) * SLAB_FLOATS;
+#pragma unroll
+        for (int i = 0; i < NIT; ++i) load_piece(i, d0 - 1 + t_first);
+#pragma unroll
+        for (int i = 0; i < NIT; ++i) stage_piece(i, d0 - 1 + t_first, buf);
+#pragma unroll
+        for (int i = 0; i < NIT; ++i) load_piece(i, d0 + t_first);
+        __syncthreads();
+    }
+
+    auto plane = [&](auto Pc, int t) __attribute__((always_inline)) {
+        const int q = d0 - 1 + t;
+        float* cur = slab + (t & 1) * SLAB_FLOATS;
+        float* nxt = slab + ((t + 1) & 1) * SLAB_FLOATS;
+        sweep(Pc, std::integral_constant<int, 7>{}, cur, s2_finish, [&](int G) __attribute__((always_inline)) { staging(G, q, nxt); });
+        if (q >= d0) {
+            const bool in_vol = q < a.D;
+            if (q & 1) {
+                if (in_vol) s2_sweep(std::false_type{}, cur);
+            } else {
+                s2_turn();
+                if (in_vol) s2_sweep(std::true_type{}, cur);
+                s2_park(q);
+            }
+        }
+        retire(Pc, q - 1);
+        __syncthreads();
+    };
+    auto first_plane = [&]() __attribute__((always_inline)) {
+        const int q = d0 - 1;
+        float* nxt = slab + SLAB_FLOATS;
+        sweep(std::integral_constant<int, 0>{}, std::integral_constant<int, 1>{}, slab, []() {},
+              [&](int G) __attribute__((always_inline)) { staging(G, q, nxt); });
+        retire(std::integral_constant<int, 0>{}, q - 1);
+        __syncthreads();
+    };
+    auto last_plane = [&](auto Pc) __attribute__((always_inline)) {
+        constexpr int P = decltype(Pc)::value;
+        const int q = d1;
+        const float* cur = slab + ((T - 1) & 1) * SLAB_FLOATS;
+        const bool in_vol = q < a.D;
+        if (in_vol) sweep(Pc, std::integral_constant<int, 1 << ((P + 1) % 3)>{}, cur, s2_finish, [](int) {});
+        else s2_finish();
+        s2_turn();
+        if (in_vol) s2_sweep(std::integral_constant<int, 2>{}, cur);
+        s2_park(q);
+        retire(Pc, q - 1);
+        __syncthreads();
+    };
+    const int t_lo = trim_first ? 1 : 0, t_hi = trim_last ? T - 1 : T;
+    if (trim_first && d0 > 0) first_plane();
+    for (int t = 0; t < t_hi; t += 3) {
+        if (t >= t_lo) plane(std::integral_constant<int, 0>{}, t);
+        if (t + 1 < t_hi) plane(std::integral_constant<int, 1>{}, t + 1);
+        if (t + 2 < t_hi) plane(std::integral_constant<int, 2>{}, t + 2);
+    }
+    if (trim_last) {
+        const int pl = (T - 1) % 3;
+        if (pl == 0) last_plane(std::integral_constant<int, 0>{});
+        else if (pl == 1) last_plane(std::integral_constant<int, 1>{});
+        else last_plane(std::integral_constant<int, 2>{});
+    }
+
+    s2_finish();
+    if (fa.stats2 && wave == 0) {
+        double* s2p = fa.stats2 + (size_t)((blockIdx.x + gridDim.x * blockIdx.z) % (fa.slots2 > 1 ? fa.slots2 : 1)) * 2 * COUT2;
+#pragma unroll
+        for (int rt = 0; rt < 2; ++rt)
+#pragma unroll
+            for (int k = 0; k < 4; ++k) {
+                float sv = st2_s[rt][k], qv = st2_q[rt][k];
+#pragma unroll
+                for (int o = 8; o > 0; o >>= 1) { sv += __shfl_xor(sv, o, 64); qv += __shfl_xor(qv, o, 64); }
+                if (n == 0) {
+                    atomicAdd(&s2p[16 * rt + 4 * kq + k], (double)sv);
+                    atomicAdd(&s2p[COUT2 + 16 * rt + 4 * kq + k], (double)qv);
+                }
+            }
+    }
+    __syncthreads();
+
+    if (a.stats) stats_commit<COUT>(st_s, st_q, false, slab, conv_stats_row(a), a.cout_total, 0);
+}
+
+}
+
+int mvs_conv_s1_wino_weight_layout(const float* w, float* out, hipStream_t st) {
+    s1_wino_weight_layout_kernel<<<mvs_cdiv(W_FLOATS, 256), 256, 0, st>>>(w, out);
+    return (int)hipGetLastError();
+}
+
+int mvs_conv3d_s1_wino_fuse2_launch(const ConvArgs& a, const float* wprep_wino, const float* w2, float* y2, double* stats2,
+                                    int full_sweeps, hipStream_t st) {
+    const WinoS1Args fa = {wprep_wino, w2, y2, stats2, a.stats_slots, full_sweeps};
+    const int tiles = ((a.H + TH - 1) / TH) * ((a.W + TW - 1) / TW);
+    const dim3 grid(tiles, 1, (a.D + a.planes_per_wg - 1) / a.planes_per_wg);
+    const size_t smem = (size_t)LDS_FLOATS * sizeof(float);
+    static bool attr_done = false;
+    if (!attr_done) {
+        hipError_t e = hipFuncSetAttribute((const void*)conv3d_s1_wino_kernel, hipFuncAttributeMaxDynamicSharedMemorySize, (int)smem);
+        if (e != hipSuccess) return (int)e;
+        attr_done = true;
+    }
+    conv3d_s1_wino_kernel<<<grid, 256, smem, st>>>(a, fa);
+    return (int)hipGetLastError();
+}
diff --git a/mvsnet_amd/csrc/conv_common.h b/mvsnet_amd/csrc/conv_common.h
--- a/mvsnet_amd/csrc/conv_common.h
+++ b/mvsnet_amd/csrc/conv_common.h
@@ -176,7 +176,8 @@
 }
 
 int mvs_conv3d_dispatch(ConvArgs& a, int Cin, int Cout, int stride, hipStream_t st);
-int mvs_conv3d_s1_fuse2_launch(const ConvArgs& a, const float* w2, float* y2, double* stats2, hipStream_t st);
+int mvs_conv3d_s1_fuse2_launch(const ConvArgs& a, const float* w2, float* y2, double* stats2, hipStream_t st,
+                               const float* wprep_wino = nullptr);
 int mvs_conv_weight_layout(const float* w, int kind, int Cin, int Cout, float* out, hipStream_t st);
 int mvs_conv3d_scalar(const float* x, const float* xs, const float* xb, const float* x2, const float* x2s, const float* x2b,
                       const float* w, int D, int H, int W, int Cin, int Cout, int stride, float* y, double* stats, hipStream_t st);
@@ -200,6 +201,16 @@
 int mvs_conv_wino_weight_layout(const float* w, float* out, hipStream_t st);
 int mvs_conv3d_c8_wino_s2_launch(const ConvArgs& a, const float* wprep_wino, const float* w2, float* y2, double* stats2,
                                  hipStream_t st, int slots1, int slots2);
+__device__ __forceinline__ float wino_u(float g0, float g1, float g2, int pt) {
+    if (pt == 0) return g0;
+    if (pt == 3) return g2;
+    const double s = (double)g0 + (double)g2;
+    return (float)(0.5 * (pt == 1 ? s + (double)g1 : s - (double)g1));
+}
+constexpr int MVS_CONV_S1_WINO_FLOATS = 3 * 4 * 16 * 3 * 16;
+int mvs_conv_s1_wino_weight_layout(const float* w, float* out, hipStream_t st);
+int mvs_conv3d_s1_wino_fuse2_launch(const ConvArgs& a, const float* wprep_wino, const float* w2, float* y2, double* stats2,
+                                    int full_sweeps, hipStream_t st);
 bool mvs_conv3d_os_covers(int kind, int Cin, int Cout);
 int mvs_conv3d_os_weight_layout(const float* w, int kind, int Cin, int Cout, float* out, hipStream_t st);
 int mvs_conv3d_os_launch(const ConvArgs& a, int kind, int Cin, int Cout, hipStream_t st);
diff --git a/mvsnet_amd/csrc/library.hip b/mvsnet_amd/csrc/library.hip
--- a/mvsnet_amd/csrc/library.hip
+++ b/mvsnet_amd/csrc/library.hip
@@ -27,14 +27,17 @@
 #ifndef MVS_PAIR_WAVES4_DEFAULT
 #define MVS_PAIR_WAVES4_DEFAULT 0
 #endif
+#ifndef MVS_FUSE2_DIRECT_DEFAULT
+#define MVS_FUSE2_DIRECT_DEFAULT 0
+#endif
 std::atomic<int> mvs_hooks[MVS_HOOK_COUNT] = {{-1}, {0}, {0}, {0}, {0}, {128}, {1}, {0}, {0}, {0}, {0}, {0}, {0}, {0}, {0}, {0}, {0}, {MVS_PAIR_DIRECT_DEFAULT},
-                                              {MVS_PAIR_WAVES4_DEFAULT}};
+                                              {MVS_PAIR_WAVES4_DEFAULT}, {MVS_FUSE2_DIRECT_DEFAULT}};
 extern "C" int mvs_set_test_hook(int id, int value) {
     bool ok = false;
     switch (id) {
         case MVS_HOOK_CV_TILE_ROWS_LOG2: ok = value >= -1 && value <= 3; break;
         case MVS_HOOK_CONV_NO_SPAN: case MVS_HOOK_CONV_NO_FUSE2: case MVS_HOOK_GRU_ONE_STREAM: case MVS_HOOK_UNET_PERSISTENT:
-        case MVS_HOOK_REGNET_SIDE_BRANCH: case MVS_HOOK_PAIR_DIRECT: case MVS_HOOK_PAIR_WAVES4:
+        case MVS_HOOK_REGNET_SIDE_BRANCH: case MVS_HOOK_PAIR_DIRECT: case MVS_HOOK_PAIR_WAVES4: case MVS_HOOK_FUSE2_DIRECT:
             ok = value == 0 || value == 1; break;
         case MVS_HOOK_CONV_FULL_SWEEPS: ok = value >= 0 && value < 16 && (value & 3) < 3 && (value >> 2) < 3; break;
         case MVS_HOOK_UNET_GRID: ok = value >= 0 && value <= 65536; break;
diff --git a/mvsnet_amd/csrc/regnet.hip b/mvsnet_amd/csrc/regnet.hip
--- a/mvsnet_amd/csrc/regnet.hip
+++ b/mvsnet_amd/csrc/regnet.hip
@@ -44,6 +44,16 @@
     return mvs_conv3d_c8_s2_launch(conv_args(x, w1, y1, stats1, D, H, W, Cout1), w2, y2, stats2, mvs_stream(stream));
 }
 
+extern "C" int mvs_conv3d_fuse2_f32(const float* x, const float* xs, const float* xb, const float* w1, const float* w2,
+                                    int D, int H, int W, int Cin, int Cout1, int Cout2, float* y1, double* stats1,
+                                    float* y2, double* stats2, void* stream) {
+    MVS_CHECK_ARG(x && w1 && w2 && y1 && y2 && D > 0 && H > 0 && W > 0 && (xs == nullptr) == (xb == nullptr));
+    if (Cin != 16 || Cout1 != 16 || Cout2 != 32 || mvs_get_conv_impl() == MVS_CONV_IMPL_SCALAR) return MVS_E_SHAPE;
+    ConvArgs a = conv_args(x, w1, y1, stats1, D, H, W, Cout1);
+    a.xs = xs; a.xb = xb;
+    return mvs_conv3d_s1_fuse2_launch(a, w2, y2, stats2, mvs_stream(stream));
+}
+
 
 constexpr int FILL_3_0 = 250, FILL_3_1 = 500;
 
@@ -114,6 +124,7 @@
 size_t align256(size_t b) { return (b + 255) & ~(size_t)255; }
 
 size_t wino_floats(const Net& n) { return (n.ci[L01] == 32 && n.co[L01] == 8) ? (size_t)MVS_CONV_WINO_FLOATS : 0; }
+size_t wino1_floats(const Net& n) { return (n.ci[L11] == 16 && n.co[L11] == 16) ? (size_t)MVS_CONV_S1_WINO_FLOATS : 0; }
 
 RegnetWs carve(char* base, int D, int H, int W, int b) {
     const size_t v0 = (size_t)D * H * W;
@@ -143,7 +154,7 @@
 extern "C" size_t mvs_regnet_prepared_floats(int cin, int base) {
     if (cin <= 0 || base <= 0) return 0;
     const Net n = net_of(cin, base);
-    return 2 * n.wtotal + wino_floats(n);
+    return 2 * n.wtotal + wino_floats(n) + wino1_floats(n);
 }
 
 extern "C" int mvs_regnet_prepare_f32(const float* const* weights, int cin, int base, float* prepared,
@@ -160,8 +171,11 @@
             if (rc) return rc;
         }
     }
-    if (wino_floats(n)) return mvs_conv_wino_weight_layout(weights[L01], prepared + 2 * n.wtotal, mvs_stream(stream));
-    return 0;
+    int rc = 0;
+    if (wino_floats(n)) rc = mvs_conv_wino_weight_layout(weights[L01], prepared + 2 * n.wtotal, mvs_stream(stream));
+    if (!rc && wino1_floats(n))
+        rc = mvs_conv_s1_wino_weight_layout(weights[L11], prepared + 2 * n.wtotal + wino_floats(n), mvs_stream(stream));
+    return rc;
 }
 
 namespace {
@@ -205,6 +219,7 @@
     double count(int i) const { return ((double)batch * D * H * W) / (double)(1 << (3 * out_level(i))); }
     const float* wprep(int i) const { return (prepared && net.ok[i]) ? prepared + net.woff[i] : nullptr; }
     const float* wprep_wino() const { return (prepared && wino_floats(net)) ? prepared + 2 * net.wtotal : nullptr; }
+    const float* wprep_wino1() const { return (prepared && wino1_floats(net)) ? prepared + 2 * net.wtotal + wino_floats(net) : nullptr; }
     int mark(int l, int k, hipStream_t s) const { return mvs_prof_layers.mark(lp, 2 * l + k, s); }
 };
 
@@ -292,7 +307,7 @@
         const size_t wo = (size_t)bi * r.ws_floats1;
         ConvArgs a = conv_args(r.ws.y[L10] + wo, r.weights[L11], r.ws.y[L11] + wo, r.st(L11), D1, H1, W1, r.net.co[L11]);
         a.bn = r.bn_of(L10); a.wprep = r.wprep(L11); a.stats_slots = r.SL;
-        rc = mvs_conv3d_s1_fuse2_launch(a, r.weights[L20], r.ws.y[L20] + wo, r.st(L20), r.hs);
+        rc = mvs_conv3d_s1_fuse2_launch(a, r.weights[L20], r.ws.y[L20] + wo, r.st(L20), r.hs, r.wprep_wino1());
     }
     if (rc) return rc == MVS_E_SHAPE ? APART : rc;
     return r.mark(L11, 1, r.hs);
```

Result: no change. 1152 depth maps/s, median of 6 (+1.0%).
